# twke18/SPML

Hardware: AMD Instinct MI355X
Metric: images/sec (513x513) + k-means iters/sec (higher is better)
Workload: dtype f32

## Files before the change

### spml_amd/_ffi.py

```python
import ctypes
import os
import threading
from ctypes import c_char_p, c_double, c_float, c_int, c_int64, c_size_t, c_void_p

import torch

_HERE = os.path.dirname(os.path.abspath(__file__))
LIB_PATH = os.environ.get('SPML_HIP_LIB') or os.path.join(_HERE, 'lib', 'libspml_hip.so')

_lib = None
_lock = threading.Lock()

_P = c_void_p
_SIGNATURES = {
    'spml_status_string': (c_char_p, [c_int]),
    'spml_abi_version': (c_int, []),
    'spml_normalize_concat_loc_f32': (c_int, [_P, c_int, c_int, c_int, c_int, _P, _P, _P, _P, _P]),
    'spml_normalize_concat_loc_bwd_f32': (c_int, [_P, c_int, c_int, c_int, c_int, _P, _P, _P, _P, _P, _P]),
    'spml_normalize_concat_local_f32': (c_int, [_P, c_int, c_int, c_int, c_int, _P, c_int, _P, _P, _P, _P]),
    'spml_normalize_concat_local_nhwc_supported': (c_int, [c_int, c_int]),
    'spml_normalize_concat_local_nhwc_f32': (c_int, [_P, c_int, c_int, c_int, c_int, _P, c_int, _P, _P, _P, _P]),
    'spml_normalize_concat_local_nhwc_bwd_f32': (c_int, [_P, c_int, c_int, c_int, c_int, _P, c_int, _P, _P, _P,
                                                         _P, _P]),
    'spml_normalize_concat_local_bwd_f32': (c_int, [_P, c_int, c_int, c_int, c_int, _P, c_int, _P, _P, _P,
                                                    _P, _P]),
    'spml_normalize_rows_f32': (c_int, [_P, c_int64, c_int, _P, _P]),
    'spml_normalize_rows_bwd_f32': (c_int, [_P, _P, c_int64, c_int, _P, _P]),
    'spml_kmeans_init_grid_i64': (c_int, [c_int, c_int, c_int, c_int, _P, _P]),
    'spml_relabel_unique_workspace_bytes': (c_size_t, [c_int64]),
    'spml_relabel_unique_i64': (c_int, [_P, c_int64, _P, _P, c_int64, _P, _P, c_size_t, _P]),
    'spml_kmeans_workspace_bytes': (c_size_t, [c_int64, c_int, c_int, c_int, c_int64]),
    'spml_kmeans_run_f32': (c_int, [_P, c_int64, c_int, _P, c_int, c_int64, c_int, _P, c_int, _P, _P,
                                    c_int, _P, c_size_t, _P]),
    'spml_kmeans_assign_f32': (c_int, [_P, c_int64, c_int, _P, c_int, c_int64, c_int, _P, _P, c_int,
                                       _P, c_size_t, _P]),
    'spml_kmeans_fused_pass_f32': (c_int, [_P, c_int64, c_int, _P, c_int, c_int64, c_int, _P, _P, _P,
                                           c_int, _P, c_size_t, _P]),
    'spml_kmeans_preconvert_f32': (c_int, [_P, c_int64, c_int, _P, c_int, c_int64, c_int, _P, c_size_t,
                                           _P]),
    'spml_kmeans_path_name': (c_char_p, [c_int64, c_int, c_int, c_int, c_int64, c_int, c_int, c_int]),
    'spml_kmeans_profile_layout': (c_int, [c_int64, c_int, c_int, c_int, c_int64, c_int, _P, _P]),
    'spml_kmeans_run_profiled_f32': (c_int, [_P, c_int64, c_int, _P, c_int, c_int64, c_int, _P, c_int,
                                             _P, c_int, _P, c_size_t, _P, c_size_t, _P]),
    'spml_segment_sum_normalize_f32': (c_int, [_P, _P, c_int64, c_int, c_int64, _P, _P, _P]),
    'spml_segment_sum_normalize_bwd_f32': (c_int, [_P, _P, _P, c_int64, c_int, c_int64, _P, _P, c_int, _P]),
    'spml_segment_sum_det_workspace_bytes': (c_size_t, [c_int64, c_int]),
    'spml_segment_sum_normalize_det_f32': (c_int, [_P, _P, c_int64, c_int, c_int64, _P, _P, _P, c_size_t, _P]),
    'spml_set_deterministic': (c_int, [c_int]),
    'spml_get_deterministic': (c_int, []),
    'spml_build_experiment': (c_int, []),
    'spml_segsort_nll_workspace_bytes': (c_size_t, [c_int64, c_int64, c_int]),
    'spml_segsort_nll_fwd_f32': (c_int, [_P, _P, _P, c_int64, _P, _P, c_int64, c_int, c_float, c_int,
                                         _P, _P, _P, c_size_t, _P]),
    'spml_segsort_nll_bwd_f32': (c_int, [_P, _P, _P, c_int64, _P, _P, c_int64, c_int, c_float, c_int,
                                         _P, _P, _P, _P, c_int64, _P, c_size_t, _P]),
    'spml_topk_workspace_bytes': (c_size_t, [c_int64, c_int64, c_int, c_int]),
    'spml_topk_affinity_f32': (c_int, [_P, c_int64, _P, c_int64, c_int, c_int, _P, _P, _P, c_float,
                                       _P, _P, _P, c_size_t, _P]),
    'spml_affinity_workspace_bytes': (c_size_t, [c_int, c_int, c_int64]),
    'spml_affinity_transition_f32': (c_int, [_P, c_int, c_int, c_int64, c_float, c_int, _P, _P, c_size_t,
                                             _P]),
    'spml_bn_workspace_bytes': (c_size_t, [c_int64, c_int]),
    'spml_bn_act_fwd_f32': (c_int, [_P, _P, c_int64, c_int, _P, _P, _P, _P, c_float, c_float, c_int, _P, _P, _P,
                                    _P, c_size_t, _P]),
    'spml_bn_act_bwd_f32': (c_int, [_P, _P, _P, c_int64, c_int, _P, _P, _P, _P, _P, _P, _P, _P, c_size_t, _P]),
    'spml_hl8_from_f32': (c_int, [_P, c_int64, c_int, _P, c_int, _P, _P]),
    'spml_hl8_weight_transposed_f32': (c_int, [_P, c_int, c_int, c_int, _P, _P, _P]),
    'spml_conv_hl8_supported': (c_int, [c_int, c_int, c_int]),
    'spml_conv_hl8_f32': (c_int, [_P, _P, _P, _P, _P, _P, _P, c_int, c_int, c_int, c_int, c_int, c_int, c_int, _P]),
    'spml_conv_hl8_stats_layout': (c_int, [c_int, c_int, c_int, c_int, c_int, c_int, _P, _P]),
    'spml_conv_hl8_stats_f32': (c_int, [_P, _P, _P, _P, _P, _P, _P, c_int, c_int, c_int, c_int, c_int, c_int, c_int, _P]),
    'spml_bn_fwd_hl8_chunks_f32': (c_int, [_P, _P, c_int, c_int, _P, _P, c_int64, c_int, _P, _P, _P, _P, c_float, c_float,
                                           c_int, _P, _P, _P, _P, _P, _P, _P, _P, _P]),
    'spml_conv_wgrad_hl8_supported': (c_int, [c_int, c_int, c_int]),
    'spml_conv_wgrad_workspace_bytes': (c_size_t, [c_int, c_int, c_int, c_int, c_int, c_int]),
    'spml_conv_wgrad_hl8_f32': (c_int, [_P, _P, _P, _P, _P, c_int, c_int, c_int, c_int, c_int, c_int, c_int, _P,
                                        c_size_t, _P]),
    'spml_conv_wgrad_pyramid_hl8_supported': (c_int, [c_int, c_int, c_int]),
    'spml_conv_tap_gather_f32': (c_int, [_P, _P, _P, c_int, c_int, c_int, c_int, c_int, _P, _P]),
    'spml_conv_wgrad_pyramid_workspace_bytes': (c_size_t, [c_int, c_int, c_int, c_int, c_int, c_int]),
    'spml_conv_wgrad_pyramid_hl8_f32': (c_int, [_P, _P, _P, _P, _P, c_int, c_int, c_int, c_int, c_int, c_int, _P, _P,
                                                c_size_t, _P]),
    'spml_bn_stats_ext_f32': (c_int, [_P, c_int64, c_int, _P, _P, _P, _P, _P, c_size_t, _P]),
    'spml_bn_stats_ext_chunks_f32': (c_int, [_P, c_int, c_int, c_int64, c_int, _P, _P, _P, _P, _P]),
    'spml_bn_finalize_f32': (c_int, [_P, _P, c_int, c_double, c_float, c_float, _P, _P, _P, _P]),
    'spml_bn_act_apply_hl8_f32': (c_int, [_P, _P, _P, c_int64, c_int, _P, _P, _P, _P, _P, _P, c_int, _P, _P, _P, _P,
                                          _P]),
    'spml_bn_act_bwd_reduce_ext_f32': (c_int, [_P, _P, _P, _P, c_int64, c_int, _P, _P, _P, _P, _P, _P, c_size_t, _P]),
    'spml_bn_act_bwd_apply_hl8_f32': (c_int, [_P, _P, _P, _P, c_int64, c_int, _P, _P, _P, _P, _P, _P, _P, _P,
                                              c_double, _P, _P, _P, _P, _P, _P]),
    'spml_bn_fwd_hl8_f32': (c_int, [_P, _P, _P, c_int64, c_int, _P, _P, _P, _P, c_float, c_float, c_int, _P, _P, _P, _P,
                                    _P, _P, _P, _P, _P, c_size_t, _P]),
    'spml_bn_bwd_hl8_f32': (c_int, [_P, _P, _P, _P, c_int64, c_int, _P, _P, _P, _P, _P, _P, _P, _P, _P, _P, _P, _P,
                                    c_size_t, _P]),
    'spml_conv_hl8_pyramid_f32': (c_int, [_P, _P, _P, _P, _P, _P, _P, c_int, c_int, c_int, c_int, c_int, c_int, _P,
                                          _P]),
    'spml_hl8_weight_transposed_into_f32': (c_int, [_P, c_int, c_int, c_int, _P, _P, c_int, c_int, _P]),
    'spml_absmax_bound_f32': (c_int, [_P, c_int64, _P, c_int, _P]),
    'spml_hl8_weight_set_f32': (c_int, [_P, _P, _P, _P, c_int, _P, _P, _P, _P]),
    'spml_bn_finalize_ranks_f32': (c_int, [_P, c_int, c_int, c_float, c_float, _P, _P, _P, _P, _P, _P]),
    'spml_conv_hl8_affine_f32': (c_int, [_P, _P, _P, _P, _P, _P, c_int, _P, _P, c_int, c_int, c_int, c_int, c_int,
                                         c_int, c_int, _P]),
    'spml_upsample_ce_supported': (c_int, [c_int]),
    'spml_upsample_ce_workspace_bytes': (c_size_t, [c_int, c_int, c_int]),
    'spml_upsample_ce_fwd_f32': (c_int, [_P, _P, c_int, c_int, c_int, c_int, c_int, c_int, c_int64, _P, _P, _P,
                                         c_size_t, _P]),
    'spml_upsample_ce_bwd_f32': (c_int, [_P, _P, _P, c_int, c_int, c_int, c_int, c_int, c_int, c_int64, _P, _P, _P]),
    'spml_bn_stats_f32': (c_int, [_P, c_int64, c_int, _P, _P, _P, c_size_t, _P]),
    'spml_bn_act_apply_f32': (c_int, [_P, _P, c_int64, c_int, _P, _P, _P, _P, c_int, _P, _P]),
    'spml_bn_act_bwd_reduce_f32': (c_int, [_P, _P, _P, c_int64, c_int, _P, _P, _P, _P, _P, c_size_t, _P]),
    'spml_bn_act_bwd_apply_f32': (c_int, [_P, _P, _P, c_int64, c_int, _P, _P, _P, _P, _P, c_double, _P, _P, _P,
                                          _P]),
    'spml_clock_probe': (c_int, [_P, c_int, _P]),
    'spml_maxpool3x3s2_nhwc_f32': (c_int, [_P, c_int, c_int, c_int, c_int, _P, _P]),
    'spml_window_accumulate_f32': (c_int, [_P, c_int, c_int, c_int, _P, _P, c_int, c_int, c_int, c_int,
                                           _P]),
    'spml_unit_hl8_from_nchw_f32': (c_int, [_P, c_int, c_int, c_int, c_int, _P, _P]),
    'spml_class_head_supported': (c_int, [c_int, c_int]),
    'spml_class_head_accumulate_f32': (c_int, [_P, c_int, c_int, c_int, _P, _P, c_int, _P, c_int, c_int, c_int, c_int,
                                               _P]),
    'spml_argmax_channels_i64': (c_int, [_P, c_int, c_int, c_int, c_int, c_int, _P, _P]),
    'spml_iou_counts_i64': (c_int, [_P, _P, c_int64, c_int, _P, _P]),
    'spml_resample_unit_f32': (c_int, [_P, c_int, c_int, c_int, c_int64, c_int64, c_int64, c_int, c_int, c_int, c_int,
                                       c_int, _P, c_int, c_int, _P]),
    'spml_resample_classes_accumulate_f32': (c_int, [_P, c_int, c_int, c_int, c_int64, c_int64, c_int64, c_int, c_int,
                                                     c_int, c_int, c_int, c_int, _P, _P]),
    'spml_cam_finalize_f32': (c_int, [_P, c_int, c_int64, c_int, c_int, _P, c_int, c_float, _P, _P]),
    'spml_upsample_argmax_i64': (c_int, [_P, c_int, c_int, c_int, c_int, c_int, _P, _P]),
}

EXPORTS = tuple(_SIGNATURES)


class SpmlHipError(RuntimeError):
  pass


ABI_VERSION = 6


def lib():
  global _lib
  if _lib is None:
    with _lock:
      if _lib is None:
        if not os.path.exists(LIB_PATH):
          raise SpmlHipError(
              'libspml_hip.so not found at %s -- build it with `python -m spml_amd._build` '
              '(there is no CPU fallback for the HIP path)' % LIB_PATH)
        handle = ctypes.CDLL(LIB_PATH)
        for name, (res, args) in _SIGNATURES.items():
          try:
            fn = getattr(handle, name)
          except AttributeError:
            raise SpmlHipError('libspml_hip.so does not export %s (stale build? run '
                               '`python -m spml_amd._build --force`)' % name)
          fn.restype = res
          fn.argtypes = args
        got = handle.spml_abi_version()
        if got != ABI_VERSION:
          raise SpmlHipError('libspml_hip.so has ABI version %d, this wrapper was written against %d (stale build? '
                             'run `python -m spml_amd._build --force`)' % (got, ABI_VERSION))
        exp = handle.spml_build_experiment()
        want = (int(os.environ.get('SPML_CONV_EXP') or 0) & 0xffff) | ((int(os.environ.get('SPML_P64_EXP') or 0) & 0xffff) << 16)
        if exp != want:
          raise SpmlHipError('libspml_hip.so is a profiling build (SPML_CONV_EXP=%d, SPML_P64_EXP=%d: kernels that skip work '
                             'and overwrite outputs) but this process asks for (%d, %d) -- rebuild with '
                             '`python -m spml_amd._build`' % (exp & 0xffff, exp >> 16, want & 0xffff, want >> 16))
        if os.environ.get('SPML_DETERMINISTIC', '0') not in ('', '0'):
          handle.spml_set_deterministic(1)
        _lib = handle
  return _lib


def set_deterministic(on):
  return bool(lib().spml_set_deterministic(1 if on else 0))


def deterministic():
  return bool(lib().spml_get_deterministic())


def check(rc, what):
  if rc != 0:
    raise SpmlHipError('%s failed: %s (status %d)' % (
        what, lib().spml_status_string(rc).decode(), rc))


def stream_ptr():
  return c_void_p(torch.cuda.current_stream().cuda_stream)


def ptr(t, dtype=None, allow_none=False):
  if t is None:
    if allow_none:
      return c_void_p(0)
    raise SpmlHipError('missing tensor argument')
  if not t.is_cuda:
    raise SpmlHipError('the HIP path needs GPU tensors (got %s); there is no CPU fallback'
                       % t.device)
  if t.device.index != torch.cuda.current_device():
    raise SpmlHipError('tensor lives on %s but the current device is cuda:%d -- wrap the call in '
                       '`torch.cuda.device(tensor.device)`' % (t.device, torch.cuda.current_device()))
  if not t.is_contiguous():
    raise SpmlHipError('tensor must be contiguous')
  if dtype is not None and t.dtype != dtype:
    raise SpmlHipError('expected dtype %s, got %s' % (dtype, t.dtype))
  return c_void_p(t.data_ptr())


def workspace(nbytes, device):
  n = max(int(nbytes), 16)
  if n > (64 << 20):
    g = min(1 << (n.bit_length() - 4), 256 << 20)
    n = (n + g - 1) // g * g
  return torch.empty((n,), dtype=torch.uint8, device=device)



def k1_channels_last(emb, nl):
  return (emb.dim() == 4 and emb.dtype == torch.float32 and not emb.is_contiguous() and
          emb.is_contiguous(memory_format=torch.channels_last) and
          bool(lib().spml_normalize_concat_local_nhwc_supported(int(emb.shape[1]), int(nl))))


def normalize_concat_loc(emb, loc=None, row_map=None, num_rows=None, want_emb=True,
                         want_loc=True):
  n, c, h, w = emb.shape
  nl = 2 if loc is None else int(loc.shape[-1])
  rows = n * h * w if num_rows is None else int(num_rows)
  out_emb = torch.empty((rows, c), dtype=torch.float32, device=emb.device) if want_emb else None
  out_loc = torch.empty((rows, c + nl), dtype=torch.float32, device=emb.device) if want_loc else None
  if k1_channels_last(emb, nl):
    check(lib().spml_normalize_concat_local_nhwc_f32(
        _ptr_any(emb), n, c, h, w, ptr(loc, torch.float32, True), nl,
        ptr(row_map, torch.int64, True), ptr(out_emb, None, True), ptr(out_loc, None, True),
        stream_ptr()), 'spml_normalize_concat_local_nhwc_f32')
    return out_emb, out_loc
  check(lib().spml_normalize_concat_local_f32(
      ptr(emb, torch.float32), n, c, h, w, ptr(loc, torch.float32, True), nl,
      ptr(row_map, torch.int64, True), ptr(out_emb, None, True), ptr(out_loc, None, True),
      stream_ptr()), 'spml_normalize_concat_local_f32')
  return out_emb, out_loc


def normalize_concat_loc_bwd(emb, loc, row_map, d_out_emb, d_out_loc):
  n, c, h, w = emb.shape
  nl = 2 if loc is None else int(loc.shape[-1])
  d_emb = torch.empty_like(emb)
  if k1_channels_last(emb, nl):
    check(lib().spml_normalize_concat_local_nhwc_bwd_f32(
        _ptr_any(emb), n, c, h, w, ptr(loc, torch.float32, True), nl,
        ptr(row_map, torch.int64, True), ptr(d_out_emb, torch.float32, True),
        ptr(d_out_loc, torch.float32, True), _ptr_any(d_emb), stream_ptr()),
          'spml_normalize_concat_local_nhwc_bwd_f32')
    return d_emb
  check(lib().spml_normalize_concat_local_bwd_f32(
      ptr(emb, torch.float32), n, c, h, w, ptr(loc, torch.float32, True), nl,
      ptr(row_map, torch.int64, True), ptr(d_out_emb, torch.float32, True),
      ptr(d_out_loc, torch.float32, True), ptr(d_emb), stream_ptr()),
        'spml_normalize_concat_local_bwd_f32')
  return d_emb


def normalize_rows(x):
  d = x.shape[-1]
  x2 = x.reshape(-1, d)
  y = torch.empty_like(x2)
  check(lib().spml_normalize_rows_f32(ptr(x2, torch.float32), x2.shape[0], d, ptr(y),
                                      stream_ptr()), 'spml_normalize_rows_f32')
  return y.view(x.shape)


def normalize_rows_bwd(x, dy):
  d = x.shape[-1]
  x2, g2 = x.reshape(-1, d), dy.reshape(-1, d).contiguous()
  dx = torch.empty_like(x2)
  check(lib().spml_normalize_rows_bwd_f32(ptr(x2, torch.float32), ptr(g2, torch.float32),
                                          x2.shape[0], d, ptr(dx), stream_ptr()),
        'spml_normalize_rows_bwd_f32')
  return dx.view(x.shape)


def kmeans_init_grid(h, w, ky, kx, device):
  out = torch.empty((h, w), dtype=torch.int64, device=device)
  check(lib().spml_kmeans_init_grid_i64(h, w, ky, kx, ptr(out), stream_ptr()),
        'spml_kmeans_init_grid_i64')
  return out


_last_kmeans = None


def relabel_unique(keys, with_uniq=True, padded=False):
  keys = keys.reshape(-1)
  if keys.dtype != torch.int64 or not keys.is_contiguous():
    keys = keys.long().contiguous()
  p = keys.shape[0]
  inv = torch.empty((p,), dtype=torch.int64, device=keys.device)
  count = torch.empty((1,), dtype=torch.int64, device=keys.device)
  if padded:
    uniq = torch.full((p,), torch.iinfo(torch.int64).max, dtype=torch.int64, device=keys.device)
  else:
    uniq = torch.empty((p if with_uniq else 0,), dtype=torch.int64, device=keys.device)
  ws = workspace(lib().spml_relabel_unique_workspace_bytes(p), keys.device)
  check(lib().spml_relabel_unique_i64(ptr(keys, torch.int64, p == 0), p, ptr(inv, allow_none=p == 0),
                                      ptr(uniq, allow_none=uniq.numel() == 0), uniq.numel(), ptr(count), ptr(ws),
                                      ws.numel(), stream_ptr()), 'spml_relabel_unique_i64')
  if padded:
    return uniq, inv, count
  if not with_uniq:
    return None, inv, count
  return uniq[:int(count.item())], inv, count


def _note_kmeans(p, d, k, n_img, max_seg_len, iterations, given, flags):
  global _last_kmeans
  _last_kmeans = (int(p), int(d), int(k), int(n_img), int(max_seg_len), int(iterations), int(given),
                  int(flags))


def kmeans_path_name(p, d, k, n_img, max_seg_len, iterations, given_centroids=False, flags=0):
  return lib().spml_kmeans_path_name(int(p), int(d), int(k), int(n_img), int(max_seg_len),
                                     int(iterations), int(bool(given_centroids)), int(flags)).decode()


def kmeans_last_path():
  return 'none' if _last_kmeans is None else lib().spml_kmeans_path_name(*_last_kmeans).decode()


def kmeans_run(x, seg_offsets, max_seg_len, k, labels_init, iterations, want_centroids=False,
               flags=0):
  p, d = x.shape
  n_img = seg_offsets.shape[0] - 1
  labels = torch.empty((p,), dtype=torch.int64, device=x.device)
  cent = (torch.zeros((n_img, k, d), dtype=torch.float32, device=x.device)
          if want_centroids else None)
  nbytes = lib().spml_kmeans_workspace_bytes(p, d, k, n_img, max_seg_len)
  ws = workspace(nbytes, x.device)
  check(lib().spml_kmeans_run_f32(
      ptr(x, torch.float32), p, d, ptr(seg_offsets, torch.int64), n_img, int(max_seg_len), k,
      ptr(labels_init, torch.int64), int(iterations), ptr(labels), ptr(cent, None, True),
      int(flags), ptr(ws), ws.numel(), stream_ptr()), 'spml_kmeans_run_f32')
  _note_kmeans(p, d, k, n_img, max_seg_len, iterations, 0, flags)
  return (labels, cent) if want_centroids else labels


def kmeans_run_profiled(x, seg_offsets, max_seg_len, k, labels_init, iterations, flags=0):
  import ctypes
  p, d = x.shape
  n_img = seg_offsets.shape[0] - 1
  n_pass, wgs = ctypes.c_int(0), ctypes.c_int(0)
  check(lib().spml_kmeans_profile_layout(p, d, k, n_img, int(max_seg_len), int(iterations),
                                         ctypes.byref(n_pass), ctypes.byref(wgs)),
        'spml_kmeans_profile_layout')
  clocks = torch.zeros((n_pass.value, wgs.value, 2), dtype=torch.int64, device=x.device)
  labels = torch.empty((p,), dtype=torch.int64, device=x.device)
  ws = workspace(lib().spml_kmeans_workspace_bytes(p, d, k, n_img, max_seg_len), x.device)
  check(lib().spml_kmeans_run_profiled_f32(
      ptr(x, torch.float32), p, d, ptr(seg_offsets, torch.int64), n_img, int(max_seg_len), k,
      ptr(labels_init, torch.int64), int(iterations), ptr(labels), int(flags), ptr(ws), ws.numel(),
      ptr(clocks), clocks.numel(), stream_ptr()), 'spml_kmeans_run_profiled_f32')
  _note_kmeans(p, d, k, n_img, max_seg_len, iterations, 0, flags)
  c = clocks.cpu()
  start = torch.where(c[:, :, 0] == 0, torch.full_like(c[:, :, 0], torch.iinfo(torch.int64).max), c[:, :, 0])
  dur = (c[:, :, 1].max(dim=1).values - start.min(dim=1).values).double() * 0.01
  return labels, dur


def kmeans_assign(x, seg_offsets, max_seg_len, centroids, flags=0):
  p, d = x.shape
  n_img = seg_offsets.shape[0] - 1
  k = centroids.shape[-2]
  labels = torch.empty((p,), dtype=torch.int64, device=x.device)
  nbytes = lib().spml_kmeans_workspace_bytes(p, d, k, n_img, max_seg_len)
  ws = workspace(nbytes, x.device)
  check(lib().spml_kmeans_assign_f32(
      ptr(x, torch.float32), p, d, ptr(seg_offsets, torch.int64), n_img, int(max_seg_len), k,
      ptr(centroids, torch.float32), ptr(labels), int(flags), ptr(ws), ws.numel(),
      stream_ptr()), 'spml_kmeans_assign_f32')
  _note_kmeans(p, d, k, n_img, max_seg_len, 1, 1, flags)
  return labels


def kmeans_workspace(x, seg_offsets, max_seg_len, k):
  p, d = x.shape
  return workspace(lib().spml_kmeans_workspace_bytes(p, d, k, seg_offsets.shape[0] - 1, max_seg_len),
                   x.device)


def kmeans_preconvert(x, seg_offsets, max_seg_len, k, ws):
  p, d = x.shape
  check(lib().spml_kmeans_preconvert_f32(
      ptr(x, torch.float32), p, d, ptr(seg_offsets, torch.int64), seg_offsets.shape[0] - 1,
      int(max_seg_len), int(k), ptr(ws), ws.numel(), stream_ptr()), 'spml_kmeans_preconvert_f32')


def kmeans_fused_pass(x, seg_offsets, max_seg_len, centroids, ws=None, preconverted=False, flags=0,
                      out=None):
  p, d = x.shape
  n_img = seg_offsets.shape[0] - 1
  k = centroids.shape[-2]
  if ws is None:
    ws = kmeans_workspace(x, seg_offsets, max_seg_len, k)
  if out is None:
    out = (torch.empty((p,), dtype=torch.int64, device=x.device),
           torch.empty((n_img, k, d), dtype=torch.float32, device=x.device))
  labels, sums = out
  flags = int(flags) | (32 if preconverted else 0)
  check(lib().spml_kmeans_fused_pass_f32(
      ptr(x, torch.float32), p, d, ptr(seg_offsets, torch.int64), n_img, int(max_seg_len), k,
      ptr(centroids, torch.float32), ptr(labels, torch.int64), ptr(sums, torch.float32), flags,
      ptr(ws), ws.numel(), stream_ptr()), 'spml_kmeans_fused_pass_f32')
  _note_kmeans(p, d, k, n_img, max_seg_len, 1, 1, flags)
  return labels, sums


def clock_probe(device, spin_us, stream):
  out = torch.zeros((2,), dtype=torch.int64, device=device)
  stream.wait_stream(torch.cuda.current_stream(device))
  check(lib().spml_clock_probe(ptr(out), int(spin_us), c_void_p(stream.cuda_stream)), 'spml_clock_probe')
  return out


def maxpool3x3s2_nhwc(x):
  n, c, h, w = x.shape
  oh, ow = (h - 1) // 2 + 1, (w - 1) // 2 + 1
  y = torch.empty((n, c, oh, ow), dtype=torch.float32, device=x.device, memory_format=torch.channels_last)
  check(lib().spml_maxpool3x3s2_nhwc_f32(_ptr_any(x), n, h, w, c, _ptr_any(y), stream_ptr()), 'spml_maxpool3x3s2_nhwc_f32')
  return y


def segment_sum_normalize(x, ids, m):
  p, d = x.shape
  sums = torch.empty((m, d), dtype=torch.float32, device=x.device)
  protos = torch.empty((m, d), dtype=torch.float32, device=x.device)
  if deterministic():
    nbytes = lib().spml_segment_sum_det_workspace_bytes(int(m), d)
    ws = workspace(nbytes, x.device)
    check(lib().spml_segment_sum_normalize_det_f32(ptr(x, torch.float32), ptr(ids, torch.int64), p, d, int(m),
                                                   ptr(sums), ptr(protos), ptr(ws), ws.numel(), stream_ptr()),
          'spml_segment_sum_normalize_det_f32')
    return protos, sums
  check(lib().spml_segment_sum_normalize_f32(ptr(x, torch.float32), ptr(ids, torch.int64), p, d,
                                             int(m), ptr(sums), ptr(protos), stream_ptr()),
        'spml_segment_sum_normalize_f32')
  return protos, sums


def segment_sum_normalize_bwd(d_protos, sums, ids, p):
  m, d = sums.shape
  scratch = torch.empty_like(sums)
  dx = torch.empty((p, d), dtype=torch.float32, device=sums.device)
  check(lib().spml_segment_sum_normalize_bwd_f32(
      ptr(d_protos, torch.float32), ptr(sums, torch.float32), ptr(ids, torch.int64), p, d, m,
      ptr(scratch), ptr(dx), 0, stream_ptr()), 'spml_segment_sum_normalize_bwd_f32')
  return dx


def segsort_nll_fwd(emb, own, px_code, protos, pr_code, kappa, mode):
  p, d = emb.shape
  m = protos.shape[0]
  nll = torch.empty((p,), dtype=torch.float32, device=emb.device)
  stats = torch.empty((p, 4), dtype=torch.float32, device=emb.device)
  ws = workspace(lib().spml_segsort_nll_workspace_bytes(p, m, d), emb.device)
  check(lib().spml_segsort_nll_fwd_f32(
      ptr(emb, torch.float32), ptr(own, torch.int64), ptr(px_code, torch.int64), p,
      ptr(protos, torch.float32), ptr(pr_code, torch.int64), m, d, float(kappa), int(mode),
      ptr(nll), ptr(stats), ptr(ws), ws.numel(), stream_ptr()), 'spml_segsort_nll_fwd_f32')
  return nll, stats


def segsort_nll_bwd(emb, own, px_code, protos, pr_code, kappa, mode, stats, d_nll, m_grad=-1):
  p, d = emb.shape
  m = protos.shape[0]
  d_emb = torch.empty_like(emb)
  d_protos = torch.zeros_like(protos)
  ws = workspace(lib().spml_segsort_nll_workspace_bytes(p, m, d), emb.device)
  check(lib().spml_segsort_nll_bwd_f32(
      ptr(emb, torch.float32), ptr(own, torch.int64), ptr(px_code, torch.int64), p,
      ptr(protos, torch.float32), ptr(pr_code, torch.int64), m, d, float(kappa), int(mode),
      ptr(stats, torch.float32), ptr(d_nll, torch.float32), ptr(d_emb), ptr(d_protos),
      int(m_grad), ptr(ws), ws.numel(), stream_ptr()), 'spml_segsort_nll_bwd_f32')
  return d_emb, d_protos


def topk_affinity(q, protos, k, q_group=None, pr_group=None, pr_valid=None, masked_value=-2.0):
  nq, d = q.shape
  m = protos.shape[0]
  idx = torch.empty((nq, k), dtype=torch.int64, device=q.device)
  val = torch.empty((nq, k), dtype=torch.float32, device=q.device)
  ws = workspace(lib().spml_topk_workspace_bytes(nq, m, d, k), q.device)
  check(lib().spml_topk_affinity_f32(
      ptr(q, torch.float32), nq, ptr(protos, torch.float32), m, d, int(k),
      ptr(q_group, torch.int64, True), ptr(pr_group, torch.int64, True),
      ptr(pr_valid, torch.uint8, True), float(masked_value), ptr(idx), ptr(val), ptr(ws),
      ws.numel(), stream_ptr()), 'spml_topk_affinity_f32')
  return idx, val


def window_accumulate(patch, acc, counts, sh, sw):
  c, h, w = patch.shape
  big_c, big_h, big_w = acc.shape
  if big_c != c or tuple(counts.shape) != (big_h, big_w):
    raise SpmlHipError('window_accumulate: shape mismatch')
  check(lib().spml_window_accumulate_f32(
      ptr(patch, torch.float32), c, h, w, ptr(acc, torch.float32), ptr(counts, torch.float32),
      big_h, big_w, int(sh), int(sw), stream_ptr()), 'spml_window_accumulate_f32')


def unit_hl8_from_nchw(x):
  n, c, h, w = x.shape
  out = torch.empty((n * h * w * c * 4,), dtype=torch.uint8, device=x.device)
  check(lib().spml_unit_hl8_from_nchw_f32(ptr(x, torch.float32), n, c, h, w, ptr(out), stream_ptr()),
        'spml_unit_hl8_from_nchw_f32')
  return Hl8(out, torch.ones((1,), dtype=torch.float32, device=x.device), n * h * w, c)


def class_head_supported(ch, ncls):
  return bool(lib().spml_class_head_supported(int(ch), int(ncls)))


def class_head_accumulate(hidden, weight, bias, canvas, sh, sw, h, w):
  ncls, ch = weight.shape
  if hidden.numel() != h * w * ch or canvas.dim() != 3 or canvas.shape[0] != ncls or bias.numel() != ncls:
    raise SpmlHipError('class_head_accumulate: shape mismatch')
  check(lib().spml_class_head_accumulate_f32(
      _ptr_any(hidden), ch, int(h), int(w), ptr(weight, torch.float32), ptr(bias, torch.float32), ncls,
      ptr(canvas, torch.float32), canvas.shape[1], canvas.shape[2], int(sh), int(sw), stream_ptr()),
        'spml_class_head_accumulate_f32')


def argmax_channels(canvas, h, w):
  ncls, hp, wp = canvas.shape
  out = torch.empty((h, w), dtype=torch.int64, device=canvas.device)
  check(lib().spml_argmax_channels_i64(ptr(canvas, torch.float32), ncls, hp, wp, int(h), int(w), ptr(out),
                                       stream_ptr()), 'spml_argmax_channels_i64')
  return out


def iou_counts(pred, target, ncls, counts=None):
  if pred.numel() != target.numel():
    raise SpmlHipError('iou_counts: pred and target differ in size')
  if counts is None:
    counts = torch.zeros((3, ncls), dtype=torch.int64, device=pred.device)
  elif tuple(counts.shape) != (3, ncls):
    raise SpmlHipError('iou_counts: counts must be [3, num_classes]')
  check(lib().spml_iou_counts_i64(ptr(pred, torch.int64), ptr(target, torch.int64), pred.numel(), int(ncls),
                                  ptr(counts, torch.int64), stream_ptr()), 'spml_iou_counts_i64')
  return counts


COMBINE_MODES = {'prob_mean': 0, 'logit_mean': 1}


def _combine(combine):
  if combine not in COMBINE_MODES:
    raise SpmlHipError("combine must be 'prob_mean' or 'logit_mean' (got %r)" % (combine,))
  return COMBINE_MODES[combine]


def _view_args(x, crop_hw, out_hw, what):
  if x.dim() != 3:
    raise SpmlHipError('%s: expected a [C, Hp, Wp] tensor' % what)
  c, hp, wp = x.shape
  (rh, rw), (oh, ow) = crop_hw, out_hw
  if not (0 < rh <= hp and 0 < rw <= wp and oh > 0 and ow > 0):
    raise SpmlHipError('%s: crop %r / output %r do not fit a %d x %d plane' % (what, crop_hw, out_hw, hp, wp))
  sc, sy, sx = x.stride()
  return c, hp, wp, sc, sy, sx, int(rh), int(rw), int(oh), int(ow)


def resample_unit(emb, crop_hw, flip, out_hw, out, b):
  c, hp, wp, sc, sy, sx, rh, rw, oh, ow = _view_args(emb, crop_hw, out_hw, 'resample_unit')
  if out.dim() != 3 or out.shape[1] != c or out.shape[2] != oh * ow or not 0 <= b < out.shape[0]:
    raise SpmlHipError('resample_unit: out must be [B, %d, %d] with b < B' % (c, oh * ow))
  check(lib().spml_resample_unit_f32(_ptr_any(emb), c, hp, wp, sc, sy, sx, rh, rw, int(bool(flip)), oh, ow,
                                     ptr(out, torch.float32), out.shape[0], int(b), stream_ptr()),
        'spml_resample_unit_f32')
  return out


def resample_classes_accumulate(logit, crop_hw, flip, out_hw, acc, combine='prob_mean'):
  ncls, hp, wp, sc, sy, sx, rh, rw, oh, ow = _view_args(logit, crop_hw, out_hw, 'resample_classes_accumulate')
  if acc.shape[0] != ncls or acc.numel() != ncls * oh * ow:
    raise SpmlHipError('resample_classes_accumulate: acc must hold [%d, %d] values' % (ncls, oh * ow))
  check(lib().spml_resample_classes_accumulate_f32(_ptr_any(logit), ncls, hp, wp, sc, sy, sx, rh, rw, int(bool(flip)),
                                                   oh, ow, _combine(combine), ptr(acc, torch.float32), stream_ptr()),
        'spml_resample_classes_accumulate_f32')
  return acc


def cam_finalize(acc, num_views, label_tags, combine='prob_mean', background_threshold=None):
  ncls = acc.shape[0]
  if label_tags.numel() != ncls or label_tags.dtype not in (torch.bool, torch.uint8):
    raise SpmlHipError('cam_finalize: label_tags must be a bool [%d] tensor' % ncls)
  if int(num_views) < 1:
    raise SpmlHipError('cam_finalize: no views')
  cam = torch.empty_like(acc)
  tags = label_tags.view(torch.uint8) if label_tags.dtype == torch.bool else label_tags
  check(lib().spml_cam_finalize_f32(ptr(acc, torch.float32), ncls, acc.numel() // ncls, int(num_views),
                                    _combine(combine), ptr(tags, torch.uint8), int(background_threshold is not None),
                                    float(background_threshold or 0.0), ptr(cam), stream_ptr()),
        'spml_cam_finalize_f32')
  return cam


def upsample_argmax(cam, h, w):
  if cam.dim() != 3:
    raise SpmlHipError('upsample_argmax: expected [ncls, oh, ow]')
  ncls, oh, ow = cam.shape
  out = torch.empty((int(h), int(w)), dtype=torch.int64, device=cam.device)
  check(lib().spml_upsample_argmax_i64(ptr(cam, torch.float32), ncls, oh, ow, int(h), int(w), ptr(out), stream_ptr()),
        'spml_upsample_argmax_i64')
  return out


def affinity_transition(emb, scale=5.0, power=20):
  b, c, n = emb.shape
  trans = torch.empty((n, n), dtype=torch.float32, device=emb.device)
  ws = workspace(lib().spml_affinity_workspace_bytes(b, c, n), emb.device)
  check(lib().spml_affinity_transition_f32(
      ptr(emb, torch.float32), b, c, n, float(scale), int(power), ptr(trans), ptr(ws), ws.numel(),
      stream_ptr()), 'spml_affinity_transition_f32')
  return trans


def _nhwc_rows(t):
  if t.dim() == 2:
    return t.shape[0], t.shape[1]
  n, c, h, w = t.shape
  if not t.is_contiguous(memory_format=torch.channels_last):
    raise SpmlHipError('fused batch norm needs channels-last (NHWC) tensors')
  return n * h * w, c


def _ptr_any(t, allow_none=False):
  if t is None:
    if allow_none:
      return c_void_p(0)
    raise SpmlHipError('missing tensor argument')
  if not t.is_cuda or t.dtype != torch.float32:
    raise SpmlHipError('expected a float32 GPU tensor (got %s on %s)' % (t.dtype, t.device))
  if t.device.index != torch.cuda.current_device():
    raise SpmlHipError('tensor lives on %s but the current device is cuda:%d' % (t.device, torch.cuda.current_device()))
  return c_void_p(t.data_ptr())


_bn_ws = {}


def _bn_workspace(r, c, device):
  need = lib().spml_bn_workspace_bytes(r, c)
  key = (device.index, torch.cuda.current_stream().cuda_stream)
  ws = _bn_ws.get(key)
  if ws is None or ws.numel() < need:
    ws = workspace(need, device)
    _bn_ws[key] = ws
  return ws


def bn_act_fwd(x, residual, gamma, beta, running_mean, running_var, momentum, eps, relu):
  r, c = _nhwc_rows(x)
  y = torch.empty_like(x)
  stats = torch.empty((2, c), dtype=torch.float32, device=x.device)
  ws = _bn_workspace(r, c, x.device)
  check(lib().spml_bn_act_fwd_f32(
      _ptr_any(x), _ptr_any(residual, True), r, c, ptr(gamma, torch.float32), ptr(beta, torch.float32),
      ptr(running_mean, None, True), ptr(running_var, None, True), float(momentum), float(eps),
      int(bool(relu)), _ptr_any(y), c_void_p(stats[0].data_ptr()), c_void_p(stats[1].data_ptr()), ptr(ws),
      ws.numel(), stream_ptr()), 'spml_bn_act_fwd_f32')
  return y, stats[0], stats[1]


def bn_act_bwd(dy, y, x, mean, invstd, gamma, want_dx=True, want_dres=False):
  r, c = _nhwc_rows(dy)
  dx = torch.empty_like(dy) if want_dx else None
  dres = torch.empty_like(dy) if want_dres else None
  dgb = torch.empty((2, c), dtype=torch.float32, device=dy.device)
  ws = _bn_workspace(r, c, dy.device)
  check(lib().spml_bn_act_bwd_f32(
      _ptr_any(dy), _ptr_any(y, True), _ptr_any(x), r, c, c_void_p(mean.data_ptr()), c_void_p(invstd.data_ptr()),
      ptr(gamma, torch.float32), c_void_p(dgb[0].data_ptr()), c_void_p(dgb[1].data_ptr()), _ptr_any(dx, True),
      _ptr_any(dres, True), ptr(ws), ws.numel(), stream_ptr()), 'spml_bn_act_bwd_f32')
  return dx, dres, dgb[0], dgb[1]


def bn_stats(x):
  r, c = _nhwc_rows(x)
  mean = torch.empty((c,), dtype=torch.float32, device=x.device)
  m2 = torch.empty((c,), dtype=torch.float32, device=x.device)
  ws = workspace(lib().spml_bn_workspace_bytes(r, c), x.device)
  check(lib().spml_bn_stats_f32(_ptr_any(x), r, c, ptr(mean), ptr(m2), ptr(ws), ws.numel(), stream_ptr()),
        'spml_bn_stats_f32')
  return mean, m2


def bn_act_apply(x, residual, mean, invstd, gamma, beta, relu):
  r, c = _nhwc_rows(x)
  y = torch.empty_like(x)
  check(lib().spml_bn_act_apply_f32(_ptr_any(x), _ptr_any(residual, True), r, c, ptr(mean), ptr(invstd),
                                    ptr(gamma, torch.float32), ptr(beta, torch.float32), int(bool(relu)),
                                    _ptr_any(y), stream_ptr()), 'spml_bn_act_apply_f32')
  return y


def bn_act_bwd_reduce(dy, y, x, mean, invstd):
  r, c = _nhwc_rows(x)
  s0 = torch.empty((c,), dtype=torch.float32, device=x.device)
  s1 = torch.empty((c,), dtype=torch.float32, device=x.device)
  ws = workspace(lib().spml_bn_workspace_bytes(r, c), x.device)
  check(lib().spml_bn_act_bwd_reduce_f32(_ptr_any(dy), _ptr_any(y, True), _ptr_any(x), r, c, ptr(mean),
                                         ptr(invstd), ptr(s0), ptr(s1), ptr(ws), ws.numel(), stream_ptr()),
        'spml_bn_act_bwd_reduce_f32')
  return s0, s1


def bn_act_bwd_apply(dy, y, x, mean, invstd, gamma, sum_dz, sum_dz_xhat, count, want_dx=True,
                     want_dres=False):
  r, c = _nhwc_rows(dy)
  count, count_dev = _count_args(count)
  dx = torch.empty_like(dy) if want_dx else None
  dres = torch.empty_like(dy) if want_dres else None
  check(lib().spml_bn_act_bwd_apply_f32(
      _ptr_any(dy), _ptr_any(y, True), _ptr_any(x, True), r, c, ptr(mean, None, True), ptr(invstd, None, True),
      ptr(gamma, None, True), ptr(sum_dz, None, True), ptr(sum_dz_xhat, None, True), count, count_dev,
      _ptr_any(dx, True), _ptr_any(dres, True), stream_ptr()), 'spml_bn_act_bwd_apply_f32')
  return dx, dres



class Hl8(object):
  __slots__ = ('data', 'bound', 'rows', 'channels')

  def __init__(self, data, bound, rows, channels):
    self.data, self.bound, self.rows, self.channels = data, bound, rows, channels


def hl8_from_f32(x, rows=None, channels=None, bound=None):
  if rows is None:
    rows, channels = _nhwc_rows(x)
  compute = bound is None
  if compute:
    bound = torch.empty((1,), dtype=torch.float32, device=x.device)
  out = torch.empty((rows * channels * 4,), dtype=torch.uint8, device=x.device)
  check(lib().spml_hl8_from_f32(_ptr_any(x), rows, channels, c_void_p(bound.data_ptr()), int(compute),
                                ptr(out), stream_ptr()), 'spml_hl8_from_f32')
  return Hl8(out, bound, rows, channels)


def hl8_weight(w):
  cout, cin, kh, kw = w.shape
  taps = kh * kw
  wl = w.detach().contiguous(memory_format=torch.channels_last)
  fwd = hl8_from_f32(wl, cout, taps * cin)
  tr = torch.empty((cout * taps * cin * 4,), dtype=torch.uint8, device=w.device)
  check(lib().spml_hl8_weight_transposed_f32(_ptr_any(wl), cout, taps, cin, c_void_p(fwd.bound.data_ptr()),
                                             ptr(tr), stream_ptr()), 'spml_hl8_weight_transposed_f32')
  return fwd, Hl8(tr, fwd.bound, cin, taps * cout)


def conv_hl8_supported(k, n, taps):
  return bool(lib().spml_conv_hl8_supported(int(k), int(n), int(taps)))


def conv_hl8(a, b, n_img, h, w, taps, dilation=1, addend=None, addend_mask=None):
  k, n = a.channels, b.rows
  if a.rows != n_img * h * w or b.channels != taps * k:
    raise SpmlHipError('conv_hl8: operand shapes do not match')
  out = torch.empty((n_img, n, h, w), dtype=torch.float32, device=a.data.device,
                    memory_format=torch.channels_last)
  check(lib().spml_conv_hl8_f32(ptr(a.data), c_void_p(a.bound.data_ptr()), ptr(b.data),
                                c_void_p(b.bound.data_ptr()), _ptr_any(addend, True), _dp(addend_mask), _ptr_any(out),
                                n_img, h, w,
                                k, n, taps, dilation, stream_ptr()), 'spml_conv_hl8_f32')
  return out


class ChunkStats(object):

  def __init__(self, data, chunks, chunk_rows, bound):
    self.data, self.chunks, self.chunk_rows, self.bound = data, chunks, chunk_rows, bound


def conv_hl8_stats(a, b, n_img, h, w, taps, dilation=1):
  import ctypes
  k, n = a.channels, b.rows
  chunks, rows = ctypes.c_int(0), ctypes.c_int(0)
  if os.environ.get('SPML_CONV_BN_STATS') == '0' or lib().spml_conv_hl8_stats_layout(
      n_img, h, w, k, n, taps, ctypes.byref(chunks), ctypes.byref(rows)) != 0:
    return conv_hl8(a, b, n_img, h, w, taps, dilation), None
  if a.rows != n_img * h * w or b.channels != taps * k:
    raise SpmlHipError('conv_hl8_stats: operand shapes do not match')
  dev = a.data.device
  out = torch.empty((n_img, n, h, w), dtype=torch.float32, device=dev, memory_format=torch.channels_last)
  st = torch.empty((4, chunks.value, n), dtype=torch.float32, device=dev)
  bound = _f32(1, dev)
  check(lib().spml_conv_hl8_stats_f32(ptr(a.data), c_void_p(a.bound.data_ptr()), ptr(b.data),
                                      c_void_p(b.bound.data_ptr()), _ptr_any(out), _dp(st), _dp(bound), n_img, h, w,
                                      k, n, taps, dilation, stream_ptr()), 'spml_conv_hl8_stats_f32')
  return out, ChunkStats(st, chunks.value, rows.value, bound)


def conv_wgrad_hl8_supported(k, n, taps):
  return bool(lib().spml_conv_wgrad_hl8_supported(int(k), int(n), int(taps)))


_wgrad_ws = {}


def conv_wgrad_hl8(dy, x, n_img, h, w, taps, dilation=1):
  n, k = dy.channels, x.channels
  if dy.rows != n_img * h * w or x.rows != dy.rows:
    raise SpmlHipError('conv_wgrad_hl8: operand shapes do not match')
  need = lib().spml_conv_wgrad_workspace_bytes(n_img, h, w, k, n, taps)
  key = (dy.data.device.index, torch.cuda.current_stream().cuda_stream)
  ws = _wgrad_ws.get(key)
  if ws is None or ws.numel() < need:
    ws = workspace(need, dy.data.device)
    _wgrad_ws[key] = ws
  side = 3 if taps == 9 else 1
  dw = torch.empty((n, k, side, side), dtype=torch.float32, device=dy.data.device,
                   memory_format=torch.channels_last)
  check(lib().spml_conv_wgrad_hl8_f32(ptr(dy.data), c_void_p(dy.bound.data_ptr()), ptr(x.data),
                                      c_void_p(x.bound.data_ptr()), _ptr_any(dw), n_img, h, w, k, n, taps,
                                      dilation, ptr(ws), ws.numel(), stream_ptr()), 'spml_conv_wgrad_hl8_f32')
  return dw


def conv_wgrad_pyramid_hl8_supported(k, n, branches):
  return bool(lib().spml_conv_wgrad_pyramid_hl8_supported(int(k), int(n), int(branches)))


def conv_wgrad_pyramid_hl8(dy, x, n_img, h, w, dilations):
  n, k, nb = dy.channels, x.channels, len(dilations)
  if dy.rows != n_img * h * w or x.rows != dy.rows:
    raise SpmlHipError('conv_wgrad_pyramid_hl8: operand shapes do not match')
  need = lib().spml_conv_wgrad_pyramid_workspace_bytes(n_img, h, w, k, n, nb)
  if need == 0:
    raise SpmlHipError('conv_wgrad_pyramid_hl8: unsupported shape (K %d, N %d, %d branches)' % (k, n, nb))
  key = (dy.data.device.index, torch.cuda.current_stream().cuda_stream)
  ws = _wgrad_ws.get(key)
  if ws is None or ws.numel() < need:
    ws = workspace(need, dy.data.device)
    _wgrad_ws[key] = ws
  dw = torch.empty((nb, n, 3, 3, k), dtype=torch.float32, device=dy.data.device)
  dil = (ctypes.c_int * nb)(*[int(d) for d in dilations])
  check(lib().spml_conv_wgrad_pyramid_hl8_f32(ptr(dy.data), c_void_p(dy.bound.data_ptr()), ptr(x.data),
                                              c_void_p(x.bound.data_ptr()), _ptr_any(dw), n_img, h, w, k, n, nb,
                                              ctypes.cast(dil, c_void_p), ptr(ws), ws.numel(), stream_ptr()),
        'spml_conv_wgrad_pyramid_hl8_f32')
  return [dw[b].permute(0, 3, 1, 2) for b in range(nb)]


def _f32(n, device):
  return torch.empty((n,), dtype=torch.float32, device=device)


def _dp(t):
  return c_void_p(0) if t is None else c_void_p(t.data_ptr())


def bn_stats_ext(x, rows, channels, chunk_stats=None):
  st = torch.empty((5, channels), dtype=torch.float32, device=x.device)
  st[0].fill_(float(rows))
  if chunk_stats is not None:
    check(lib().spml_bn_stats_ext_chunks_f32(_dp(chunk_stats.data), chunk_stats.chunks, chunk_stats.chunk_rows, rows,
                                             channels, _dp(st[1]), _dp(st[2]), _dp(st[3]), _dp(st[4]), stream_ptr()),
          'spml_bn_stats_ext_chunks_f32')
    return st
  ws = _bn_workspace(rows, channels, x.device)
  check(lib().spml_bn_stats_ext_f32(_ptr_any(x), rows, channels, _dp(st[1]), _dp(st[2]), _dp(st[3]), _dp(st[4]),
                                    ptr(ws), ws.numel(), stream_ptr()), 'spml_bn_stats_ext_f32')
  return st


def _count_args(count):
  if torch.is_tensor(count):
    return 0.0, ptr(count, torch.float32)
  return float(count), None


def bn_finalize_ranks(gathered, eps, momentum, running_mean, running_var):
  world, _, c = gathered.shape
  out = torch.empty((2 * c + 4,), dtype=torch.float32, device=gathered.device)
  mean, invstd, total = out[:c], out[c:2 * c], out[2 * c:2 * c + 1]
  check(lib().spml_bn_finalize_ranks_f32(ptr(gathered, torch.float32), world, c, float(eps), float(momentum),
                                         _dp(running_mean), _dp(running_var), _dp(mean), _dp(invstd), _dp(total),
                                         stream_ptr()),
        'spml_bn_finalize_ranks_f32')
  return mean, invstd, total


def bn_finalize(mean, m2, count, eps, momentum, running_mean, running_var):
  invstd = torch.empty_like(mean)
  check(lib().spml_bn_finalize_f32(_dp(mean), _dp(m2), mean.numel(), float(count), float(eps), float(momentum),
                                   _dp(running_mean), _dp(running_var), _dp(invstd), stream_ptr()),
        'spml_bn_finalize_f32')
  return invstd


def bn_act_apply_hl8(x, rows, channels, residual, residual_bound, mean, invstd, gamma, beta, cmax, cmin, relu,
                     want_f32, want_hl8, like=None, want_mask=False):
  y = torch.empty_like(x if like is None else like) if want_f32 else None
  yh = torch.empty((rows * channels * 4,), dtype=torch.uint8, device=x.device) if want_hl8 else None
  bound = _f32(1, x.device)
  mask = torch.empty((rows * (channels // 4),), dtype=torch.uint8, device=x.device) if want_mask else None
  check(lib().spml_bn_act_apply_hl8_f32(
      _ptr_any(x), _ptr_any(residual, True), _dp(residual_bound), rows, channels, _dp(mean), _dp(invstd),
      ptr(gamma, torch.float32), ptr(beta, torch.float32), _dp(cmax), _dp(cmin), int(bool(relu)), _ptr_any(y, True),
      _dp(yh), _dp(bound), _dp(mask), stream_ptr()), 'spml_bn_act_apply_hl8_f32')
  return y, (Hl8(yh, bound, rows, channels) if want_hl8 else None), bound, mask


def bn_act_bwd_reduce_ext(dy, y, relu_mask, x, rows, channels, mean, invstd):
  st = torch.empty((3, channels), dtype=torch.float32, device=dy.device)
  ws = _bn_workspace(rows, channels, dy.device)
  check(lib().spml_bn_act_bwd_reduce_ext_f32(
      _ptr_any(dy), _ptr_any(y, True), _dp(relu_mask), _ptr_any(x), rows, channels,
      _dp(mean), _dp(invstd), _dp(st[0]), _dp(st[1]), _dp(st[2]), ptr(ws), ws.numel(), stream_ptr()),
        'spml_bn_act_bwd_reduce_ext_f32')
  return st


def bn_act_bwd_apply_hl8(dy, y, relu_mask, x, rows, channels, mean, invstd, gamma, s0, s1, max_dz, cmax, cmin, count,
                         want_dx_f32=False, want_dx_hl8=True, want_dres=False):
  dx = torch.empty_like(dy) if want_dx_f32 else None
  dxh = torch.empty((rows * channels * 4,), dtype=torch.uint8, device=dy.device) if want_dx_hl8 else None
  bound = _f32(1, dy.device) if want_dx_hl8 else None
  dres = torch.empty_like(dy) if want_dres else None
  count, count_dev = _count_args(count)
  check(lib().spml_bn_act_bwd_apply_hl8_f32(
      _ptr_any(dy), _ptr_any(y, True), _dp(relu_mask), _ptr_any(x), rows, channels,
      _dp(mean), _dp(invstd), ptr(gamma, torch.float32), _dp(s0), _dp(s1), _dp(max_dz), _dp(cmax), _dp(cmin),
      count, count_dev, _ptr_any(dx, True), _dp(dxh), _dp(bound), _ptr_any(dres, True), stream_ptr()),
        'spml_bn_act_bwd_apply_hl8_f32')
  return dx, (Hl8(dxh, bound, rows, channels) if want_dx_hl8 else None), dres


def bn_fwd_hl8(x, rows, channels, residual, residual_bound, gamma, beta, running_mean, running_var, momentum, eps,
               relu, want_f32, want_hl8, want_mask, chunk_stats=None):
  y = torch.empty_like(x) if want_f32 else None
  yh = torch.empty((rows * channels * 4,), dtype=torch.uint8, device=x.device) if want_hl8 else None
  bound = _f32(1, x.device) if chunk_stats is None else chunk_stats.bound
  mask = torch.empty((rows * (channels // 4),), dtype=torch.uint8, device=x.device) if want_mask else None
  st = torch.empty((4, channels), dtype=torch.float32, device=x.device)
  if chunk_stats is not None:
    check(lib().spml_bn_fwd_hl8_chunks_f32(
        _ptr_any(x), _dp(chunk_stats.data), chunk_stats.chunks, chunk_stats.chunk_rows, _ptr_any(residual, True),
        _dp(residual_bound), rows, channels, ptr(gamma, torch.float32), ptr(beta, torch.float32), _dp(running_mean),
        _dp(running_var), float(momentum), float(eps), int(bool(relu)), _ptr_any(y, True), _dp(yh), _dp(bound),
        _dp(mask), _dp(st[0]), _dp(st[1]), _dp(st[2]), _dp(st[3]), stream_ptr()), 'spml_bn_fwd_hl8_chunks_f32')
    return y, (Hl8(yh, bound, rows, channels) if want_hl8 else None), bound, mask, (st[0], st[1], st[2], st[3])
  ws = _bn_workspace(rows, channels, x.device)
  check(lib().spml_bn_fwd_hl8_f32(
      _ptr_any(x), _ptr_any(residual, True), _dp(residual_bound), rows, channels, ptr(gamma, torch.float32),
      ptr(beta, torch.float32), _dp(running_mean), _dp(running_var), float(momentum), float(eps), int(bool(relu)),
      _ptr_any(y, True), _dp(yh), _dp(bound), _dp(mask), _dp(st[0]), _dp(st[1]), _dp(st[2]), _dp(st[3]), ptr(ws),
      ws.numel(), stream_ptr()), 'spml_bn_fwd_hl8_f32')
  return y, (Hl8(yh, bound, rows, channels) if want_hl8 else None), bound, mask, (st[0], st[1], st[2], st[3])


def bn_bwd_hl8(dy, relu_mask, x, rows, channels, saved, gamma, want_dres=False):
  mean, invstd, cmax, cmin = saved
  dxh = torch.empty((rows * channels * 4,), dtype=torch.uint8, device=dy.device)
  bound = _f32(1, dy.device)
  dres = torch.empty_like(dy) if want_dres else None
  dgb = torch.empty((2, channels), dtype=torch.float32, device=dy.device)
  ws = _bn_workspace(rows, channels, dy.device)
  check(lib().spml_bn_bwd_hl8_f32(
      _ptr_any(dy), c_void_p(0), _dp(relu_mask), _ptr_any(x), rows, channels, _dp(mean), _dp(invstd),
      ptr(gamma, torch.float32), _dp(cmax), _dp(cmin), _dp(dgb[0]), _dp(dgb[1]), c_void_p(0), _dp(dxh), _dp(bound),
      _ptr_any(dres, True), ptr(ws), ws.numel(), stream_ptr()), 'spml_bn_bwd_hl8_f32')
  return Hl8(dxh, bound, rows, channels), dres, dgb[0], dgb[1]


def conv_hl8_pyramid_dgrad(dy, weights, dilations, n_img, h, w):
  groups = len(weights)
  cout, cin = weights[0].shape[0], weights[0].shape[1]
  dev = dy.data.device
  bound = torch.empty((1,), dtype=torch.float32, device=dev)
  wl = [wt.detach().contiguous(memory_format=torch.channels_last) for wt in weights]
  for g, wt in enumerate(wl):
    check(lib().spml_absmax_bound_f32(_ptr_any(wt), wt.numel(), _dp(bound), int(g == 0), stream_ptr()),
          'spml_absmax_bound_f32')
  b = torch.empty((cin * 9 * groups * cout * 4,), dtype=torch.uint8, device=dev)
  for g, wt in enumerate(wl):
    check(lib().spml_hl8_weight_transposed_into_f32(_ptr_any(wt), cout, 9, cin, _dp(bound), ptr(b), 9 * groups, 9 * g,
                                                    stream_ptr()), 'spml_hl8_weight_transposed_into_f32')
  out = torch.empty((n_img, cin, h, w), dtype=torch.float32, device=dev, memory_format=torch.channels_last)
  import ctypes
  dil = (ctypes.c_int * 4)(*([int(d) for d in dilations] + [1] * (4 - groups)))
  check(lib().spml_conv_hl8_pyramid_f32(ptr(dy.data), _dp(dy.bound), ptr(b), _dp(bound), c_void_p(0), c_void_p(0),
                                        _ptr_any(out), n_img, h, w, cout, cin, groups, dil, stream_ptr()),
        'spml_conv_hl8_pyramid_f32')
  return out


def conv_hl8_pyramid_forward(x, weights, biases, dilations, n_img, h, w):
  import ctypes
  groups = len(weights)
  cout, cin = weights[0].shape[0], weights[0].shape[1]
  dev = x.data.device
  cat = torch.cat([wt.detach().permute(0, 2, 3, 1).reshape(cout, 9 * cin) for wt in weights], dim=1).contiguous()
  b = hl8_from_f32(cat, cout, 9 * groups * cin)
  bias = None
  if any(bb is not None for bb in biases):
    bias = sum(bb.detach() for bb in biases if bb is not None).contiguous()
  out = torch.empty((n_img, cout, h, w), dtype=torch.float32, device=dev, memory_format=torch.channels_last)
  dil = (ctypes.c_int * 4)(*([int(d) for d in dilations] + [1] * (4 - groups)))
  check(lib().spml_conv_hl8_pyramid_f32(ptr(x.data), _dp(x.bound), ptr(b.data), _dp(b.bound), _dp(bias), c_void_p(0),
                                        _ptr_any(out), n_img, h, w, cin, cout, groups, dil, stream_ptr()),
        'spml_conv_hl8_pyramid_f32')
  return out


_pyramid_operand_cache = {}


def conv_hl8_pyramid_forward_gemm_supported(cin, cout, groups):
  return (16 <= cout <= 1024 and cout & (cout - 1) == 0 and 1 <= groups <= 4 and
          conv_hl8_supported(cin, 9 * groups * cout, 1))


def conv_hl8_pyramid_forward_gemm(x, weights, biases, dilations, n_img, h, w):
  import ctypes
  groups = len(weights)
  cout, cin = weights[0].shape[0], weights[0].shape[1]
  dev = x.data.device
  import weakref
  refs, vers = _pyramid_operand_cache.get('refs', ()), _pyramid_operand_cache.get('versions', ())
  if (len(refs) == groups and all(r() is wt for r, wt in zip(refs, weights)) and
      vers == tuple(wt._version for wt in weights)):
    operand = _pyramid_operand_cache['operand']
  else:
    cat = torch.stack([wt.detach().permute(2, 3, 0, 1).reshape(9 * cout, cin) for wt in weights]).reshape(
        9 * groups * cout, cin).contiguous()
    operand = hl8_from_f32(cat, 9 * groups * cout, cin)
    _pyramid_operand_cache.update(refs=tuple(weakref.ref(wt) for wt in weights),
                                  versions=tuple(wt._version for wt in weights), operand=operand)
  z = conv_hl8(x, operand, n_img, h, w, 1)
  bias = None
  if any(bb is not None for bb in biases):
    bias = sum(bb.detach() for bb in biases if bb is not None).contiguous()
  out = torch.empty((n_img, cout, h, w), dtype=torch.float32, device=dev, memory_format=torch.channels_last)
  dil = (ctypes.c_int * groups)(*[int(d) for d in dilations])
  check(lib().spml_conv_tap_gather_f32(_ptr_any(z), _dp(bias), _ptr_any(out), n_img, h, w, cout, groups,
                                       ctypes.cast(dil, c_void_p), stream_ptr()), 'spml_conv_tap_gather_f32')
  return out


def hl8_weight_set(weights):
  import ctypes
  n = len(weights)
  dev = weights[0].device
  wl = [wt.detach().contiguous(memory_format=torch.channels_last) for wt in weights]
  bounds = torch.empty((4,), dtype=torch.float32, device=dev)
  shapes = [(wt.shape[0], wt.shape[1], wt.shape[2] * wt.shape[3]) for wt in wl]
  fwd = [torch.empty((co * ci * t * 4,), dtype=torch.uint8, device=dev) for co, ci, t in shapes]
  tr = [torch.empty((co * ci * t * 4,), dtype=torch.uint8, device=dev) for co, ci, t in shapes]
  pv, iv = ctypes.c_void_p * n, ctypes.c_int * n
  check(lib().spml_hl8_weight_set_f32(
      pv(*[wt.data_ptr() for wt in wl]), iv(*[sh[0] for sh in shapes]), iv(*[sh[1] for sh in shapes]),
      iv(*[sh[2] for sh in shapes]), n, _dp(bounds), pv(*[t.data_ptr() for t in fwd]),
      pv(*[t.data_ptr() for t in tr]), stream_ptr()), 'spml_hl8_weight_set_f32')
  out = []
  for i, (co, ci, t) in enumerate(shapes):
    b = bounds[i:i + 1]
    out.append((Hl8(fwd[i], b, co, t * ci), Hl8(tr[i], b, ci, t * co)))
  return out


def conv_hl8_affine(a, b, bias, n_img, h, w, taps, dilation=1, addend=None, relu=True, want_hl8=True):
  k, n = a.channels, b.rows
  if a.rows != n_img * h * w or b.channels != taps * k:
    raise SpmlHipError('conv_hl8_affine: operand shapes do not match')
  dev = a.data.device
  out = torch.empty((n_img, n, h, w), dtype=torch.float32, device=dev, memory_format=torch.channels_last)
  bound = _f32(1, dev) if want_hl8 else None
  check(lib().spml_conv_hl8_affine_f32(ptr(a.data), _dp(a.bound), ptr(b.data), _dp(b.bound), ptr(bias, torch.float32),
                                       _ptr_any(addend, True), int(bool(relu)), _ptr_any(out), _dp(bound), n_img, h, w,
                                       k, n, taps, dilation, stream_ptr()), 'spml_conv_hl8_affine_f32')
  return out, (hl8_from_f32(out, bound=bound) if want_hl8 else None)


def upsample_ce_supported(c):
  return bool(lib().spml_upsample_ce_supported(int(c)))


def upsample_ce_fwd(logits_nhwc, labels, ignore_index):
  n, h, w, c = logits_nhwc.shape
  hh, ww = labels.shape[-2:]
  lse = torch.empty((n, hh, ww), dtype=torch.float32, device=logits_nhwc.device)
  result = torch.empty((3,), dtype=torch.float32, device=logits_nhwc.device)
  ws = workspace(lib().spml_upsample_ce_workspace_bytes(n, hh, ww), logits_nhwc.device)
  check(lib().spml_upsample_ce_fwd_f32(ptr(logits_nhwc, torch.float32), ptr(labels, torch.int64), n, c, h, w, hh, ww,
                                       int(ignore_index), ptr(lse), ptr(result), ptr(ws), ws.numel(), stream_ptr()),
        'spml_upsample_ce_fwd_f32')
  return result, lse


def upsample_ce_bwd(logits_nhwc, labels, lse, ignore_index, scale):
  n, h, w, c = logits_nhwc.shape
  hh, ww = labels.shape[-2:]
  d = torch.empty_like(logits_nhwc)
  check(lib().spml_upsample_ce_bwd_f32(ptr(logits_nhwc, torch.float32), ptr(labels, torch.int64),
                                       ptr(lse, torch.float32), n, c, h, w, hh, ww, int(ignore_index),
                                       ptr(scale, torch.float32), ptr(d), stream_ptr()), 'spml_upsample_ce_bwd_f32')
  return d
```

### spml_amd/csrc/bn_act.hip

```cpp
#include "common.hpp"

namespace spml {
namespace {


__device__ __forceinline__ float4v relu_mask_bits(float4v dz, const unsigned char* __restrict__ mask, size_t row,
                                                  int C, int q) {
  const unsigned m = mask[row * (size_t)(C >> 2) + q];
#pragma unroll
  for (int e = 0; e < 4; ++e) dz[e] = (m >> e) & 1u ? dz[e] : 0.f;
  return dz;
}

__device__ __forceinline__ float bn_pow2_scale(float bound) {
  if (!(bound > 0.f) || bound > 1e38f) return 1.f;
  int e;
  (void)frexpf(bound, &e);
  e = 14 - e;
  e = e < -100 ? -100 : (e > 100 ? 100 : e);
  return ldexpf(1.f, e);
}

__device__ __forceinline__ void store_hl8_quad(uint2* __restrict__ out, size_t row, int C, int q, float4v v,
                                               float s) {
  union { uint2 u; _Float16 h[4]; } hh, ll;
#pragma unroll
  for (int e = 0; e < 4; ++e) {
    const float x = v[e] * s;
    const _Float16 h = (_Float16)x;
    hh.h[e] = h;
    ll.h[e] = (_Float16)(x - (float)h);
  }
  const bool odd = (q & 1) != 0;
  const uint2 send = odd ? hh.u : ll.u;
  uint2 recv;
  recv.x = (unsigned)__shfl_xor((int)send.x, 1, kWave);
  recv.y = (unsigned)__shfl_xor((int)send.y, 1, kWave);
  uint4 unit;
  if (odd) { unit.x = recv.x; unit.y = recv.y; unit.z = ll.u.x; unit.w = ll.u.y; }
  else { unit.x = hh.u.x; unit.y = hh.u.y; unit.z = recv.x; unit.w = recv.y; }
  reinterpret_cast<uint4*>(out)[(row * (size_t)(C >> 3) + (q >> 1)) * 2 + (odd ? 1 : 0)] = unit;
}

template <int MODE, int MASK>
__global__ __launch_bounds__(256) void bn_partial(const float* __restrict__ x, const float* __restrict__ dy,
                                                  const float* __restrict__ y, const float* __restrict__ mean,
                                                  int64_t R, int C, int cq, int chunk_rows,
                                                  float* __restrict__ pa, float* __restrict__ pb,
                                                  const unsigned char* __restrict__ yh, float* __restrict__ pc,
                                                  float* __restrict__ pd, float* __restrict__ zero_me) {
  if (zero_me && blockIdx.x == 0 && blockIdx.y == 0 && threadIdx.x == 0) *zero_me = 0.f;
  __shared__ float4v sa[256], sb[256];
  const int tx = threadIdx.x % cq, ty = threadIdx.x / cq, nty = 256 / cq;
  const int q = blockIdx.x * cq + tx;
  const int64_t r0 = (int64_t)blockIdx.y * chunk_rows;
  const int nrows = (int)min((int64_t)chunk_rows, R - r0);
  const int cquads = C >> 2;
  float4v a = {0.f, 0.f, 0.f, 0.f}, b = {0.f, 0.f, 0.f, 0.f};
  float4v mu = {0.f, 0.f, 0.f, 0.f};
  float4v hi = {-3.4e38f, -3.4e38f, -3.4e38f, -3.4e38f}, lo = {3.4e38f, 3.4e38f, 3.4e38f, 3.4e38f};
  if (MODE == 1) hi = a;
  if (q < cquads) {
    mu = MODE == 1 ? *reinterpret_cast<const float4v*>(mean + 4 * q)
                   : *reinterpret_cast<const float4v*>(x + (size_t)r0 * C + 4 * q);
#pragma unroll 4
    for (int r = ty; r < nrows; r += nty) {
      const size_t o = (size_t)(r0 + r) * C + 4 * q;
      const float4v xv = *reinterpret_cast<const float4v*>(x + o);
      if (MODE == 0) {
        const float4v d = xv - mu;
        a += d;
        b += d * d;
#pragma unroll
        for (int e = 0; e < 4; ++e) { hi[e] = fmaxf(hi[e], xv[e]); lo[e] = fminf(lo[e], xv[e]); }
      } else {
        float4v dz = *reinterpret_cast<const float4v*>(dy + o);
        if (MASK == 1) {
          const float4v yv = *reinterpret_cast<const float4v*>(y + o);
#pragma unroll
          for (int e = 0; e < 4; ++e) dz[e] = yv[e] > 0.f ? dz[e] : 0.f;
        } else if (MASK == 2) {
          dz = relu_mask_bits(dz, yh, (size_t)(r0 + r), C, q);
        }
        a += dz;
        b += dz * (xv - mu);
#pragma unroll
        for (int e = 0; e < 4; ++e) hi[e] = fmaxf(hi[e], fabsf(dz[e]));
      }
    }
  }
  sa[threadIdx.x] = a;
  sb[threadIdx.x] = b;
  __syncthreads();
  if (ty == 0 && q < cquads) {
    for (int i = 1; i < nty; ++i) { a += sa[i * cq + tx]; b += sb[i * cq + tx]; }
    if (MODE == 0) {
      const float inv = 1.0f / (float)nrows;
      const float4v m = a * inv;
      b = b - m * m * (float)nrows;
#pragma unroll
      for (int e = 0; e < 4; ++e) b[e] = fmaxf(b[e], 0.f);
      a = m + mu;
    }
    *reinterpret_cast<float4v*>(pa + (size_t)blockIdx.y * C + 4 * q) = a;
    *reinterpret_cast<float4v*>(pb + (size_t)blockIdx.y * C + 4 * q) = b;
  }
  if (pc) {
    __syncthreads();
    sa[threadIdx.x] = hi;
    sb[threadIdx.x] = lo;
    __syncthreads();
    if (ty == 0 && q < cquads) {
      for (int i = 1; i < nty; ++i) {
#pragma unroll
        for (int e = 0; e < 4; ++e) {
          hi[e] = fmaxf(hi[e], sa[i * cq + tx][e]);
          lo[e] = fminf(lo[e], sb[i * cq + tx][e]);
        }
      }
      *reinterpret_cast<float4v*>(pc + (size_t)blockIdx.y * C + 4 * q) = hi;
      if (MODE == 0) *reinterpret_cast<float4v*>(pd + (size_t)blockIdx.y * C + 4 * q) = lo;
    }
  }
}

struct BnFinal { int fin; float eps, momentum; float* running_mean; float* running_var; };
struct BnBound {
  float* bound;
  const float* res_bound;
  const float* gamma;
  const float* beta;
  const float* mean;
  const float* cmax;
  const float* cmin;
  float inv_count;
};
constexpr int kMergeLanes = 64, kMergeCh = 4;

__device__ inline float merge_lanes(float v, float* sh, int tx, int ty) {
  __syncthreads();
  sh[ty * kMergeCh + tx] = v;
  __syncthreads();
  float t = 0.f;
#pragma unroll 16
  for (int i = 0; i < kMergeLanes; ++i) t += sh[i * kMergeCh + tx];
  return t;
}

template <int MODE>
__global__ __launch_bounds__(kMergeCh * kMergeLanes) void bn_merge(
    const float* __restrict__ pa, const float* __restrict__ pb, int64_t R, int C, int chunks, int chunk_rows,
    const float* __restrict__ invstd, float* __restrict__ out_a, float* __restrict__ out_b, BnFinal f,
    const float* __restrict__ pc, const float* __restrict__ pd, float* __restrict__ out_c,
    float* __restrict__ out_d, BnBound bb) {
  __shared__ float sh[kMergeCh * kMergeLanes];
  __shared__ float sh_bound[kMergeCh];
  const int tx = threadIdx.x % kMergeCh, ty = threadIdx.x / kMergeCh;
  const int n_live = min(kMergeCh, C - (int)blockIdx.x * kMergeCh);
  auto publish_bound = [&](float v) {
    sh_bound[tx] = v;
    __builtin_amdgcn_wave_barrier();
    if (tx == 0) {
      unsigned m = __float_as_uint(v);
      for (int i = 1; i < n_live; ++i) m = max(m, __float_as_uint(sh_bound[i]));
      atomicMax(reinterpret_cast<unsigned*>(bb.bound), m);
    }
  };
  const int c = min(blockIdx.x * kMergeCh + tx, C - 1);
  const bool live = blockIdx.x * kMergeCh + tx < C && ty == 0;
  float hi = -3.4e38f, lo = 3.4e38f;
  constexpr int kMergeRegs = 16;
  const bool in_regs = chunks <= kMergeRegs * kMergeLanes;
  const bool ext = pc && out_c;
  float ra[kMergeRegs], rb[kMergeRegs], rc[kMergeRegs], rd[kMergeRegs];
  if (in_regs) {
#pragma unroll
    for (int j = 0; j < kMergeRegs; ++j) {
      const int i = ty + j * kMergeLanes;
      const bool ok = i < chunks;
      const size_t o = (size_t)(ok ? i : 0) * C + c;
      ra[j] = ok ? pa[o] : 0.f;
      rb[j] = ok ? pb[o] : 0.f;
      rc[j] = (ok && ext) ? pc[o] : -3.4e38f;
      rd[j] = (ok && ext && MODE == 0) ? pd[o] : 3.4e38f;
    }
  }
  float p_gamma = 0.f, p_beta = 0.f, p_res = 0.f, p_rm = 0.f, p_rv = 0.f, p_is = 0.f, p_mu = 0.f, p_cmax = 0.f, p_cmin = 0.f;
  if (live) {
    if (MODE == 0) {
      if (f.fin && bb.bound) { p_gamma = bb.gamma[c]; p_beta = bb.beta[c]; p_res = bb.res_bound ? *bb.res_bound : 0.f; }
      if (f.fin && f.running_mean) { p_rm = f.running_mean[c]; p_rv = f.running_var[c]; }
    } else {
      p_is = invstd[c];
      if (bb.bound) { p_mu = bb.mean[c]; p_cmax = bb.cmax[c]; p_cmin = bb.cmin[c]; p_gamma = bb.gamma[c]; }
    }
  }
  if (ext) {
    if (in_regs) {
#pragma unroll
      for (int j = 0; j < kMergeRegs; ++j) {
        hi = fmaxf(hi, rc[j]);
        if (MODE == 0) lo = fminf(lo, rd[j]);
      }
    } else {
#pragma unroll 4
      for (int i = ty; i < chunks; i += kMergeLanes) {
        hi = fmaxf(hi, pc[(size_t)i * C + c]);
        if (MODE == 0) lo = fminf(lo, pd[(size_t)i * C + c]);
      }
    }
    __syncthreads();
    sh[ty * kMergeCh + tx] = hi;
    __syncthreads();
    for (int i = 0; i < kMergeLanes; ++i) hi = fmaxf(hi, sh[i * kMergeCh + tx]);
    if (MODE == 0) {
      __syncthreads();
      sh[ty * kMergeCh + tx] = lo;
      __syncthreads();
      for (int i = 0; i < kMergeLanes; ++i) lo = fminf(lo, sh[i * kMergeCh + tx]);
    }
    if (live) {
      out_c[c] = hi;
      if (MODE == 0) out_d[c] = lo;
    }
  }
  if (MODE == 0) {
    float sm = 0.f;
    if (in_regs) {
#pragma unroll
      for (int j = 0; j < kMergeRegs; ++j) {
        const int i = ty + j * kMergeLanes;
        if (i < chunks) {
          const float nb = (float)min((int64_t)chunk_rows, R - (int64_t)i * chunk_rows);
          sm += ra[j] * nb;
        }
      }
    } else {
#pragma unroll 4
      for (int i = ty; i < chunks; i += kMergeLanes) {
        const float nb = (float)min((int64_t)chunk_rows, R - (int64_t)i * chunk_rows);
        sm += pa[(size_t)i * C + c] * nb;
      }
    }
    const float m = merge_lanes(sm, sh, tx, ty) / (float)R;
    float m2 = 0.f;
    if (in_regs) {
#pragma unroll
      for (int j = 0; j < kMergeRegs; ++j) {
        const int i = ty + j * kMergeLanes;
        if (i < chunks) {
          const float nb = (float)min((int64_t)chunk_rows, R - (int64_t)i * chunk_rows);
          const float d = ra[j] - m;
          m2 += rb[j] + d * d * nb;
        }
      }
    } else {
#pragma unroll 4
      for (int i = ty; i < chunks; i += kMergeLanes) {
        const float nb = (float)min((int64_t)chunk_rows, R - (int64_t)i * chunk_rows);
        const float d = pa[(size_t)i * C + c] - m;
        m2 += pb[(size_t)i * C + c] + d * d * nb;
      }
    }
    m2 = merge_lanes(m2, sh, tx, ty);
    if (!live) return;
    out_a[c] = m;
    if (f.fin) {
      const float is = 1.0f / sqrtf(m2 / (float)R + f.eps);
      out_b[c] = is;
      if (bb.bound) {
        const float sc = p_gamma * is, b = p_beta;
        const float v = fmaxf(fabsf((hi - m) * sc + b), fabsf((lo - m) * sc + b)) * 1.0001f + p_res;
        publish_bound(v);
      }
      if (f.running_mean) {
        f.running_mean[c] = (1.f - f.momentum) * p_rm + f.momentum * m;
        f.running_var[c] = (1.f - f.momentum) * p_rv +
                           f.momentum * (m2 / (float)(R > 1 ? R - 1 : 1));
      }
    } else {
      out_b[c] = m2;
    }
  } else {
    float s0 = 0.f, s1 = 0.f;
    if (in_regs) {
#pragma unroll
      for (int j = 0; j < kMergeRegs; ++j)
        if (ty + j * kMergeLanes < chunks) { s0 += ra[j]; s1 += rb[j]; }
    } else {
      for (int i = ty; i < chunks; i += kMergeLanes) { s0 += pa[(size_t)i * C + c]; s1 += pb[(size_t)i * C + c]; }
    }
    s0 = merge_lanes(s0, sh, tx, ty);
    s1 = merge_lanes(s1, sh, tx, ty);
    if (!live) return;
    out_a[c] = s0;
    out_b[c] = s1 * p_is;
    if (bb.bound) {
      const float is = p_is, mu = p_mu;
      const float xh = fmaxf(fabsf(p_cmax - mu), fabsf(p_cmin - mu)) * is;
      const float v = fabsf(p_gamma * is) *
                      (hi + fabsf(s0) * bb.inv_count + xh * fabsf(s1 * is) * bb.inv_count) * 1.0001f;
      publish_bound(v);
    }
  }
}


template <bool HAS_RES>
__global__ __launch_bounds__(256) void bn_apply(const float* __restrict__ x, const float* __restrict__ res,
                                                int64_t R, int C, int cq, int apply_rows,
                                                const float* __restrict__ mean,
                                                const float* __restrict__ invstd,
                                                const float* __restrict__ gamma,
                                                const float* __restrict__ beta, int relu,
                                                float* __restrict__ y, uint2* __restrict__ yh,
                                                const float* __restrict__ ybound,
                                                unsigned char* __restrict__ mask) {
  const int tx = threadIdx.x % cq, ty = threadIdx.x / cq, nty = 256 / cq;
  const int q = blockIdx.x * cq + tx;
  if (q >= (C >> 2)) return;
  const float ys = yh ? bn_pow2_scale(*ybound) : 1.f;
  const float4v mu = *reinterpret_cast<const float4v*>(mean + 4 * q);
  const float4v sc = *reinterpret_cast<const float4v*>(invstd + 4 * q) *
                     *reinterpret_cast<const float4v*>(gamma + 4 * q);
  const float4v sh = *reinterpret_cast<const float4v*>(beta + 4 * q);
  const int64_t r0 = (int64_t)blockIdx.y * apply_rows;
  const int64_t r1 = min(R, r0 + apply_rows);
#pragma unroll 4
  for (int64_t r = r0 + ty; r < r1; r += nty) {
    const size_t o = (size_t)r * C + 4 * q;
    float4v v = (*reinterpret_cast<const float4v*>(x + o) - mu) * sc + sh;
    if (HAS_RES) v += *reinterpret_cast<const float4v*>(res + o);
    if (relu) {
#pragma unroll
      for (int e = 0; e < 4; ++e) v[e] = fmaxf(v[e], 0.f);
    }
    if (y) *reinterpret_cast<float4v*>(y + o) = v;
    if (yh) store_hl8_quad(yh, (size_t)r, C, q, v, ys);
    if (mask)
      mask[(size_t)r * (C >> 2) + q] = (unsigned char)((v[0] > 0.f) | ((v[1] > 0.f) << 1) | ((v[2] > 0.f) << 2) |
                                                       ((v[3] > 0.f) << 3));
  }
}

template <int MASK>
__global__ __launch_bounds__(256) void bn_bwd_apply(const float* __restrict__ dy, const float* __restrict__ y,
                                                    const float* __restrict__ x, int64_t R, int C, int cq,
                                                    int apply_rows, const float* __restrict__ mean,
                                                    const float* __restrict__ invstd,
                                                    const float* __restrict__ gamma,
                                                    const float* __restrict__ sum_dz,
                                                    const float* __restrict__ sum_dz_xhat, float inv_count,
                                                    const float* __restrict__ count_dev,
                                                    float* __restrict__ dx, float* __restrict__ dres,
                                                    const unsigned char* __restrict__ yh, uint2* __restrict__ dxh,
                                                    const float* __restrict__ dxbound) {
  const int tx = threadIdx.x % cq, ty = threadIdx.x / cq, nty = 256 / cq;
  const int q = blockIdx.x * cq + tx;
  if (q >= (C >> 2)) return;
  if (count_dev) inv_count = 1.f / count_dev[0];
  const float ds = dxh ? bn_pow2_scale(*dxbound) : 1.f;
  float4v mu = {0.f, 0.f, 0.f, 0.f}, is = mu, gi = mu, c0 = mu, c1 = mu;
  if (dx || dxh) {
    mu = *reinterpret_cast<const float4v*>(mean + 4 * q);
    is = *reinterpret_cast<const float4v*>(invstd + 4 * q);
    gi = *reinterpret_cast<const float4v*>(gamma + 4 * q) * is;
    c0 = *reinterpret_cast<const float4v*>(sum_dz + 4 * q) * inv_count;
    c1 = *reinterpret_cast<const float4v*>(sum_dz_xhat + 4 * q) * inv_count;
  }
  const int64_t r0 = (int64_t)blockIdx.y * apply_rows;
  const int64_t r1 = min(R, r0 + apply_rows);
#pragma unroll 4
  for (int64_t r = r0 + ty; r < r1; r += nty) {
    const size_t o = (size_t)r * C + 4 * q;
    float4v dz = *reinterpret_cast<const float4v*>(dy + o);
    if (MASK == 1) {
      const float4v yv = *reinterpret_cast<const float4v*>(y + o);
#pragma unroll
      for (int e = 0; e < 4; ++e) dz[e] = yv[e] > 0.f ? dz[e] : 0.f;
    } else if (MASK == 2) {
      dz = relu_mask_bits(dz, yh, (size_t)r, C, q);
    }
    if (dres) *reinterpret_cast<float4v*>(dres + o) = dz;
    if (dx || dxh) {
      const float4v xh = (*reinterpret_cast<const float4v*>(x + o) - mu) * is;
      const float4v g = gi * (dz - c0 - xh * c1);
      if (dx) *reinterpret_cast<float4v*>(dx + o) = g;
      if (dxh) store_hl8_quad(dxh, (size_t)r, C, q, g, ds);
    }
  }
}

__device__ __forceinline__ float block_max_256(float v, float* sh) {
#pragma unroll
  for (int o = 32; o > 0; o >>= 1) v = fmaxf(v, __shfl_xor(v, o, kWave));
  if ((threadIdx.x & 63) == 0) sh[threadIdx.x >> 6] = v;
  __syncthreads();
  return fmaxf(fmaxf(sh[0], sh[1]), fmaxf(sh[2], sh[3]));
}

__global__ __launch_bounds__(256) void bn_bound_fwd(int C, const float* __restrict__ cmax,
                                                    const float* __restrict__ cmin,
                                                    const float* __restrict__ mean,
                                                    const float* __restrict__ invstd,
                                                    const float* __restrict__ gamma,
                                                    const float* __restrict__ beta,
                                                    const float* __restrict__ res_bound, float* __restrict__ out) {
  __shared__ float sh[4];
  float m = 0.f;
  for (int c = threadIdx.x; c < C; c += 256) {
    const float sc = gamma[c] * invstd[c];
    m = fmaxf(m, fmaxf(fabsf((cmax[c] - mean[c]) * sc + beta[c]), fabsf((cmin[c] - mean[c]) * sc + beta[c])));
  }
  m = block_max_256(m, sh);
  if (threadIdx.x == 0) out[0] = m * 1.0001f + (res_bound ? res_bound[0] : 0.f);
}

__global__ __launch_bounds__(256) void bn_bound_bwd(int C, const float* __restrict__ max_dz,
                                                    const float* __restrict__ cmax,
                                                    const float* __restrict__ cmin,
                                                    const float* __restrict__ mean,
                                                    const float* __restrict__ invstd,
                                                    const float* __restrict__ gamma,
                                                    const float* __restrict__ sum_dz,
                                                    const float* __restrict__ sum_dz_xhat, float inv_count,
                                                    const float* __restrict__ count_dev,
                                                    float* __restrict__ out) {
  __shared__ float sh[4];
  float m = 0.f;
  if (count_dev) inv_count = 1.f / count_dev[0];
  for (int c = threadIdx.x; c < C; c += 256) {
    const float xh = fmaxf(fabsf(cmax[c] - mean[c]), fabsf(cmin[c] - mean[c])) * invstd[c];
    m = fmaxf(m, fabsf(gamma[c] * invstd[c]) *
                     (max_dz[c] + fabsf(sum_dz[c]) * inv_count + xh * fabsf(sum_dz_xhat[c]) * inv_count));
  }
  m = block_max_256(m, sh);
  if (threadIdx.x == 0) out[0] = m * 1.0001f;
}

__global__ __launch_bounds__(256) void bn_finalize(int C, const float* __restrict__ mean,
                                                   const float* __restrict__ m2, float count, float eps,
                                                   float momentum, float* __restrict__ running_mean,
                                                   float* __restrict__ running_var, float* __restrict__ invstd) {
  const int c = blockIdx.x * 256 + threadIdx.x;
  if (c >= C) return;
  invstd[c] = 1.0f / sqrtf(m2[c] / count + eps);
  if (running_mean) {
    running_mean[c] = (1.f - momentum) * running_mean[c] + momentum * mean[c];
    running_var[c] = (1.f - momentum) * running_var[c] + momentum * (m2[c] / (count > 1.f ? count - 1.f : 1.f));
  }
}

__global__ __launch_bounds__(256) void bn_finalize_ranks(int C, int world, const float* __restrict__ stats,
                                                         float eps, float momentum,
                                                         float* __restrict__ running_mean,
                                                         float* __restrict__ running_var,
                                                         float* __restrict__ mean_out,
                                                         float* __restrict__ invstd,
                                                         float* __restrict__ total_out) {
  const int c = blockIdx.x * 256 + threadIdx.x;
  if (c >= C) return;
  float total = 0.f, sm = 0.f;
  for (int r = 0; r < world; ++r) {
    const float n = stats[((size_t)r * 3 + 0) * C + c];
    total += n;
    sm += n * stats[((size_t)r * 3 + 1) * C + c];
  }
  const float m = sm / total;
  float m2 = 0.f;
  for (int r = 0; r < world; ++r) {
    const float n = stats[((size_t)r * 3 + 0) * C + c];
    const float d = stats[((size_t)r * 3 + 1) * C + c] - m;
    m2 += stats[((size_t)r * 3 + 2) * C + c] + d * d * n;
  }
  mean_out[c] = m;
  invstd[c] = 1.0f / sqrtf(m2 / total + eps);
  if (total_out && c == 0) total_out[0] = total;
  if (running_mean) {
    running_mean[c] = (1.f - momentum) * running_mean[c] + momentum * m;
    running_var[c] = (1.f - momentum) * running_var[c] + momentum * (m2 / (total > 1.f ? total - 1.f : 1.f));
  }
}

inline int bn_cq(int C);
inline int bn_apply_rows(int64_t R, int C);
inline int bn_cq(int C) { const int q = C >> 2; return q >= 64 ? 64 : (q >= 32 ? 32 : (q >= 16 ? 16 : (q >= 8 ? 8 : 4))); }
inline int bn_chunk_rows(int64_t R, int C) {
  const int cq = bn_cq(C), col_blocks = ((C >> 2) + cq - 1) / cq;
  const int64_t target = std::min<int64_t>(1024, std::max<int64_t>(1, 1024 / col_blocks));
  return (int)std::max<int64_t>(128, (R + target - 1) / target);
}
inline int bn_chunks(int64_t R, int C) { const int cr = bn_chunk_rows(R, C); return (int)((R + cr - 1) / cr); }
inline int bn_apply_rows(int64_t R, int C) {
  const int cq = bn_cq(C), col_blocks = ((C >> 2) + cq - 1) / cq, nty = 256 / cq;
  const int64_t rows = (R * col_blocks + 4095) / 4096;
  return (int)std::min<int64_t>(256, std::max<int64_t>(nty, (rows + nty - 1) / nty * nty));
}
inline bool bn_ok(const void* p) { return (reinterpret_cast<uintptr_t>(p) & 15) == 0; }

}
}

using namespace spml;

#define SPML_BN_BY_MASK(KERNEL, MASK, ...)                                        \
  do {                                                                            \
    if ((MASK) == 1) hipLaunchKernelGGL((KERNEL<1>), __VA_ARGS__);                \
    else if ((MASK) == 2) hipLaunchKernelGGL((KERNEL<2>), __VA_ARGS__);           \
    else hipLaunchKernelGGL((KERNEL<0>), __VA_ARGS__);                            \
  } while (0)
#define SPML_BN_PARTIAL1(MASK, ...)                                               \
  do {                                                                            \
    if ((MASK) == 1) hipLaunchKernelGGL((bn_partial<1, 1>), __VA_ARGS__);         \
    else if ((MASK) == 2) hipLaunchKernelGGL((bn_partial<1, 2>), __VA_ARGS__);    \
    else hipLaunchKernelGGL((bn_partial<1, 0>), __VA_ARGS__);                     \
  } while (0)
#define SPML_BN_APPLY(HAS_RES, ...)                                               \
  do {                                                                            \
    if (HAS_RES) hipLaunchKernelGGL((bn_apply<true>), __VA_ARGS__);               \
    else hipLaunchKernelGGL((bn_apply<false>), __VA_ARGS__);                      \
  } while (0)

extern "C" size_t spml_bn_workspace_bytes(int64_t R, int C) {
  if (R <= 0 || C <= 0) return 0;
  return (size_t)4 * bn_chunks(R, C) * C * 4 + 256;
}

extern "C" int spml_bn_stats_f32(const float* x, int64_t R, int C, float* mean, float* m2, void* ws,
                                 size_t ws_bytes, void* stream) {
  if (!x || !mean || !m2 || R <= 0 || C <= 0) return SPML_ERR_INVALID_ARG;
  if ((C & 3) || !bn_ok(x) || !bn_ok(mean) || !bn_ok(m2)) return SPML_ERR_UNSUPPORTED;
  if (!ws || ws_bytes < spml_bn_workspace_bytes(R, C)) return SPML_ERR_WORKSPACE;
  const int chunks = bn_chunks(R, C), cq = bn_cq(C), crows = bn_chunk_rows(R, C);
  float* pa = static_cast<float*>(ws);
  float* pb = pa + (size_t)chunks * C;
  hipStream_t s = (hipStream_t)stream;
  hipLaunchKernelGGL((bn_partial<0, 0>), dim3(((C >> 2) + cq - 1) / cq, chunks), dim3(256), 0, s, x,
                     (const float*)nullptr, (const float*)nullptr, (const float*)nullptr, R, C, cq, crows, pa, pb, (const unsigned char*)nullptr, (float*)nullptr, (float*)nullptr, (float*)nullptr);
  hipLaunchKernelGGL(bn_merge<0>, dim3((C + kMergeCh - 1) / kMergeCh), dim3(kMergeCh * kMergeLanes), 0, s, pa, pb, R, C, chunks, crows,
                     (const float*)nullptr, mean, m2, BnFinal{0, 0.f, 0.f, nullptr, nullptr}, (const float*)nullptr, (const float*)nullptr, (float*)nullptr, (float*)nullptr, BnBound{});
  return launch_status();
}

extern "C" int spml_bn_act_apply_f32(const float* x, const float* residual, int64_t R, int C,
                                     const float* mean, const float* invstd, const float* gamma,
                                     const float* beta, int relu, float* y, void* stream) {
  if (!x || !mean || !invstd || !gamma || !beta || !y || R <= 0 || C <= 0) return SPML_ERR_INVALID_ARG;
  if ((C & 3) || !bn_ok(x) || !bn_ok(y) || (residual && !bn_ok(residual)) || !bn_ok(mean) ||
      !bn_ok(invstd) || !bn_ok(gamma) || !bn_ok(beta))
    return SPML_ERR_UNSUPPORTED;
  const int cq = bn_cq(C), arows = bn_apply_rows(R, C);
  const dim3 grid(((C >> 2) + cq - 1) / cq, (unsigned)((R + arows - 1) / arows));
  SPML_BN_APPLY(residual != nullptr, grid, dim3(256), 0, (hipStream_t)stream, x, residual, R, C, cq, arows, mean, invstd,
                     gamma, beta, relu, y, (uint2*)nullptr, (const float*)nullptr, (unsigned char*)nullptr);
  return launch_status();
}

extern "C" int spml_bn_act_bwd_reduce_f32(const float* dy, const float* y, const float* x, int64_t R,
                                          int C, const float* mean, const float* invstd,
                                          float* sum_dz, float* sum_dz_xhat, void* ws, size_t ws_bytes,
                                          void* stream) {
  if (!dy || !x || !mean || !invstd || !sum_dz || !sum_dz_xhat || R <= 0 || C <= 0)
    return SPML_ERR_INVALID_ARG;
  if ((C & 3) || !bn_ok(dy) || !bn_ok(x) || (y && !bn_ok(y)) || !bn_ok(mean)) return SPML_ERR_UNSUPPORTED;
  if (!ws || ws_bytes < spml_bn_workspace_bytes(R, C)) return SPML_ERR_WORKSPACE;
  const int chunks = bn_chunks(R, C), cq = bn_cq(C), crows = bn_chunk_rows(R, C);
  float* pa = static_cast<float*>(ws);
  float* pb = pa + (size_t)chunks * C;
  hipStream_t s = (hipStream_t)stream;
  SPML_BN_PARTIAL1(y ? 1 : 0, dim3(((C >> 2) + cq - 1) / cq, chunks), dim3(256), 0, s, x, dy, y, mean, R, C, cq, crows,
                   pa, pb, (const unsigned char*)nullptr, (float*)nullptr, (float*)nullptr, (float*)nullptr);
  hipLaunchKernelGGL(bn_merge<1>, dim3((C + kMergeCh - 1) / kMergeCh), dim3(kMergeCh * kMergeLanes), 0, s, pa, pb, R, C, chunks, crows, invstd, sum_dz,
                     sum_dz_xhat, BnFinal{0, 0.f, 0.f, nullptr, nullptr}, (const float*)nullptr, (const float*)nullptr, (float*)nullptr, (float*)nullptr, BnBound{});
  return launch_status();
}

extern "C" int spml_bn_act_bwd_apply_f32(const float* dy, const float* y, const float* x, int64_t R,
                                         int C, const float* mean, const float* invstd,
                                         const float* gamma, const float* sum_dz,
                                         const float* sum_dz_xhat, double count,
                                         const float* count_dev, float* dx,
                                         float* d_residual, void* stream) {
  if (!dy || R <= 0 || C <= 0 || (!dx && !d_residual) || (count <= 0 && !count_dev)) return SPML_ERR_INVALID_ARG;
  if (dx && (!x || !mean || !invstd || !gamma || !sum_dz || !sum_dz_xhat)) return SPML_ERR_INVALID_ARG;
  if ((C & 3) || !bn_ok(dy) || (y && !bn_ok(y)) || (dx && !bn_ok(dx)) || (d_residual && !bn_ok(d_residual)))
    return SPML_ERR_UNSUPPORTED;
  const int cq = bn_cq(C), arows = bn_apply_rows(R, C);
  const dim3 grid(((C >> 2) + cq - 1) / cq, (unsigned)((R + arows - 1) / arows));
  SPML_BN_BY_MASK(bn_bwd_apply, y ? 1 : 0, grid, dim3(256), 0, (hipStream_t)stream, dy, y, x, R, C, cq, arows, mean, invstd,
                     gamma, sum_dz, sum_dz_xhat, count > 0 ? (float)(1.0 / count) : 0.f, count_dev, dx, d_residual,
                     (const unsigned char*)nullptr, (uint2*)nullptr, (const float*)nullptr);
  return launch_status();
}

extern "C" int spml_bn_act_fwd_f32(const float* x, const float* residual, int64_t R, int C,
                                   const float* gamma, const float* beta, float* running_mean,
                                   float* running_var, float momentum, float eps, int relu, float* y,
                                   float* mean, float* invstd, void* ws, size_t ws_bytes,
                                   void* stream) {
  if (!x || !gamma || !beta || !y || !mean || !invstd || R <= 0 || C <= 0) return SPML_ERR_INVALID_ARG;
  if ((C & 3) || !bn_ok(x) || !bn_ok(y) || (residual && !bn_ok(residual)) || !bn_ok(mean) ||
      !bn_ok(invstd) || !bn_ok(gamma) || !bn_ok(beta))
    return SPML_ERR_UNSUPPORTED;
  if (!ws || ws_bytes < spml_bn_workspace_bytes(R, C)) return SPML_ERR_WORKSPACE;
  const int chunks = bn_chunks(R, C), cq = bn_cq(C), crows = bn_chunk_rows(R, C), arows = bn_apply_rows(R, C);
  float* pa = static_cast<float*>(ws);
  float* pb = pa + (size_t)chunks * C;
  hipStream_t s = (hipStream_t)stream;
  hipLaunchKernelGGL((bn_partial<0, 0>), dim3(((C >> 2) + cq - 1) / cq, chunks), dim3(256), 0, s, x,
                     (const float*)nullptr, (const float*)nullptr, (const float*)nullptr, R, C, cq, crows, pa, pb, (const unsigned char*)nullptr, (float*)nullptr, (float*)nullptr, (float*)nullptr);
  hipLaunchKernelGGL(bn_merge<0>, dim3((C + kMergeCh - 1) / kMergeCh), dim3(kMergeCh * kMergeLanes), 0, s, pa, pb, R, C, chunks, crows,
                     (const float*)nullptr, mean, invstd, BnFinal{1, eps, momentum, running_mean, running_var}, (const float*)nullptr, (const float*)nullptr, (float*)nullptr, (float*)nullptr, BnBound{});
  const dim3 grid(((C >> 2) + cq - 1) / cq, (unsigned)((R + arows - 1) / arows));
  SPML_BN_APPLY(residual != nullptr, grid, dim3(256), 0, s, x, residual, R, C, cq, arows, mean, invstd, gamma, beta, relu, y, (uint2*)nullptr, (const float*)nullptr, (unsigned char*)nullptr);
  return launch_status();
}

extern "C" int spml_bn_act_bwd_f32(const float* dy, const float* y, const float* x, int64_t R, int C,
                                   const float* mean, const float* invstd, const float* gamma,
                                   float* d_gamma, float* d_beta, float* dx, float* d_residual,
                                   void* ws, size_t ws_bytes, void* stream) {
  if (!dy || !x || !mean || !invstd || !gamma || !d_gamma || !d_beta || R <= 0 || C <= 0)
    return SPML_ERR_INVALID_ARG;
  int rc = spml_bn_act_bwd_reduce_f32(dy, y, x, R, C, mean, invstd, d_beta, d_gamma, ws, ws_bytes, stream);
  if (rc != SPML_OK) return rc;
  if (!dx && !d_residual) return SPML_OK;
  return spml_bn_act_bwd_apply_f32(dy, y, x, R, C, mean, invstd, gamma, d_beta, d_gamma, (double)R, nullptr, dx,
                                   d_residual, stream);
}

extern "C" int spml_bn_stats_ext_f32(const float* x, int64_t R, int C, float* mean, float* m2, float* cmax,
                                     float* cmin, void* ws, size_t ws_bytes, void* stream) {
  if (!x || !mean || !m2 || !cmax || !cmin || R <= 0 || C <= 0) return SPML_ERR_INVALID_ARG;
  if ((C & 3) || !bn_ok(x) || !bn_ok(mean) || !bn_ok(m2)) return SPML_ERR_UNSUPPORTED;
  if (!ws || ws_bytes < spml_bn_workspace_bytes(R, C)) return SPML_ERR_WORKSPACE;
  const int chunks = bn_chunks(R, C), cq = bn_cq(C), crows = bn_chunk_rows(R, C);
  float* pa = static_cast<float*>(ws);
  float* pb = pa + (size_t)chunks * C;
  float* pc = pb + (size_t)chunks * C;
  float* pd = pc + (size_t)chunks * C;
  hipStream_t s = (hipStream_t)stream;
  hipLaunchKernelGGL((bn_partial<0, 0>), dim3(((C >> 2) + cq - 1) / cq, chunks), dim3(256), 0, s, x,
                     (const float*)nullptr, (const float*)nullptr, (const float*)nullptr, R, C, cq, crows, pa, pb,
                     (const unsigned char*)nullptr, pc, pd, (float*)nullptr);
  hipLaunchKernelGGL(bn_merge<0>, dim3((C + kMergeCh - 1) / kMergeCh), dim3(kMergeCh * kMergeLanes), 0, s, pa, pb, R, C, chunks, crows,
                     (const float*)nullptr, mean, m2, BnFinal{0, 0.f, 0.f, nullptr, nullptr}, (const float*)pc,
                     (const float*)pd, cmax, cmin, BnBound{});
  return launch_status();
}

extern "C" int spml_bn_stats_ext_chunks_f32(const float* chunk_stats, int chunks, int chunk_rows, int64_t R, int C,
                                            float* mean, float* m2, float* cmax, float* cmin, void* stream) {
  if (!chunk_stats || !mean || !m2 || !cmax || !cmin || R <= 0 || C <= 0 || chunks <= 0 || chunk_rows <= 0 ||
      (int64_t)chunks * chunk_rows < R || (int64_t)(chunks - 1) * chunk_rows >= R)
    return SPML_ERR_INVALID_ARG;
  const float* pa = chunk_stats;
  const float* pb = pa + (size_t)chunks * C;
  const float* pc = pb + (size_t)chunks * C;
  const float* pd = pc + (size_t)chunks * C;
  hipLaunchKernelGGL(bn_merge<0>, dim3((C + kMergeCh - 1) / kMergeCh), dim3(kMergeCh * kMergeLanes), 0,
                     (hipStream_t)stream, pa, pb, R, C, chunks, chunk_rows, (const float*)nullptr, mean, m2,
                     BnFinal{0, 0.f, 0.f, nullptr, nullptr}, pc, pd, cmax, cmin, BnBound{});
  return launch_status();
}

extern "C" int spml_bn_finalize_f32(const float* mean, const float* m2, int C, double count, float eps,
                                    float momentum, float* running_mean, float* running_var, float* invstd,
                                    void* stream) {
  if (!mean || !m2 || !invstd || C <= 0 || count <= 0) return SPML_ERR_INVALID_ARG;
  hipLaunchKernelGGL(bn_finalize, dim3((C + 255) / 256), dim3(256), 0, (hipStream_t)stream, C, mean, m2,
                     (float)count, eps, momentum, running_mean, running_var, invstd);
  return launch_status();
}

extern "C" int spml_bn_act_apply_hl8_f32(const float* x, const float* residual, const float* residual_bound,
                                         int64_t R, int C, const float* mean, const float* invstd,
                                         const float* gamma, const float* beta, const float* cmax,
                                         const float* cmin, int relu, float* y, void* y_hl8, float* y_bound,
                                         unsigned char* relu_mask, void* stream) {
  if (!x || !mean || !invstd || !gamma || !beta || (!y && !y_hl8) || R <= 0 || C <= 0) return SPML_ERR_INVALID_ARG;
  if ((y_hl8 || y_bound) && (!cmax || !cmin || !y_bound || (residual && !residual_bound))) return SPML_ERR_INVALID_ARG;
  if ((C & 7) || !bn_ok(x) || (y && !bn_ok(y)) || (y_hl8 && !bn_ok(y_hl8)) || (residual && !bn_ok(residual)) ||
      !bn_ok(mean) || !bn_ok(invstd) || !bn_ok(gamma) || !bn_ok(beta))
    return SPML_ERR_UNSUPPORTED;
  hipStream_t s = (hipStream_t)stream;
  if (y_bound)
    hipLaunchKernelGGL(bn_bound_fwd, dim3(1), dim3(256), 0, s, C, cmax, cmin, mean, invstd, gamma, beta,
                       residual ? residual_bound : (const float*)nullptr, y_bound);
  const int cq = bn_cq(C), arows = bn_apply_rows(R, C);
  const dim3 grid(((C >> 2) + cq - 1) / cq, (unsigned)((R + arows - 1) / arows));
  SPML_BN_APPLY(residual != nullptr, grid, dim3(256), 0, s, x, residual, R, C, cq, arows, mean, invstd, gamma, beta, relu, y,
                static_cast<uint2*>(y_hl8), (const float*)y_bound, relu_mask);
  return launch_status();
}

extern "C" int spml_bn_act_bwd_reduce_ext_f32(const float* dy, const float* y, const unsigned char* relu_mask,
                                              const float* x,
                                              int64_t R, int C, const float* mean, const float* invstd,
                                              float* sum_dz, float* sum_dz_xhat, float* max_dz, void* ws,
                                              size_t ws_bytes, void* stream) {
  if (!dy || !x || !mean || !invstd || !sum_dz || !sum_dz_xhat || !max_dz || R <= 0 || C <= 0)
    return SPML_ERR_INVALID_ARG;
  if ((C & 7) || !bn_ok(dy) || !bn_ok(x) || (y && !bn_ok(y)) || !bn_ok(mean)) return SPML_ERR_UNSUPPORTED;
  if (!ws || ws_bytes < spml_bn_workspace_bytes(R, C)) return SPML_ERR_WORKSPACE;
  const int chunks = bn_chunks(R, C), cq = bn_cq(C), crows = bn_chunk_rows(R, C);
  float* pa = static_cast<float*>(ws);
  float* pb = pa + (size_t)chunks * C;
  float* pc = pb + (size_t)chunks * C;
  hipStream_t s = (hipStream_t)stream;
  SPML_BN_PARTIAL1(y ? 1 : (relu_mask ? 2 : 0), dim3(((C >> 2) + cq - 1) / cq, chunks), dim3(256), 0, s, x, dy, y, mean,
                   R, C, cq, crows, pa, pb, relu_mask, pc, (float*)nullptr, (float*)nullptr);
  hipLaunchKernelGGL(bn_merge<1>, dim3((C + kMergeCh - 1) / kMergeCh), dim3(kMergeCh * kMergeLanes), 0, s, pa, pb, R, C, chunks, crows,
                     invstd, sum_dz, sum_dz_xhat, BnFinal{0, 0.f, 0.f, nullptr, nullptr}, (const float*)pc,
                     (const float*)nullptr, max_dz, (float*)nullptr, BnBound{});
  return launch_status();
}

extern "C" int spml_bn_act_bwd_apply_hl8_f32(const float* dy, const float* y, const unsigned char* relu_mask,
                                             const float* x,
                                             int64_t R, int C, const float* mean, const float* invstd,
                                             const float* gamma, const float* sum_dz, const float* sum_dz_xhat,
                                             const float* max_dz, const float* cmax, const float* cmin,
                                             double count, const float* count_dev, float* dx, void* dx_hl8,
                                             float* dx_bound, float* d_residual, void* stream) {
  if (!dy || R <= 0 || C <= 0 || (!dx && !dx_hl8 && !d_residual) || (count <= 0 && !count_dev))
    return SPML_ERR_INVALID_ARG;
  const float inv_count = count > 0 ? (float)(1.0 / count) : 0.f;
  if ((dx || dx_hl8) && (!x || !mean || !invstd || !gamma || !sum_dz || !sum_dz_xhat)) return SPML_ERR_INVALID_ARG;
  if (dx_hl8 && (!max_dz || !cmax || !cmin || !dx_bound)) return SPML_ERR_INVALID_ARG;
  if ((C & 7) || !bn_ok(dy) || (y && !bn_ok(y)) || (dx && !bn_ok(dx)) ||
      (dx_hl8 && !bn_ok(dx_hl8)) || (d_residual && !bn_ok(d_residual)))
    return SPML_ERR_UNSUPPORTED;
  hipStream_t s = (hipStream_t)stream;
  if (dx_hl8)
    hipLaunchKernelGGL(bn_bound_bwd, dim3(1), dim3(256), 0, s, C, max_dz, cmax, cmin, mean, invstd, gamma, sum_dz,
                       sum_dz_xhat, inv_count, count_dev, dx_bound);
  const int cq = bn_cq(C), arows = bn_apply_rows(R, C);
  const dim3 grid(((C >> 2) + cq - 1) / cq, (unsigned)((R + arows - 1) / arows));
  SPML_BN_BY_MASK(bn_bwd_apply, y ? 1 : (relu_mask ? 2 : 0), grid, dim3(256), 0, s, dy, y, x, R, C, cq, arows, mean, invstd, gamma, sum_dz,
                     sum_dz_xhat, inv_count, count_dev, dx, d_residual, relu_mask,
                  static_cast<uint2*>(dx_hl8), (const float*)dx_bound);
  return launch_status();
}

extern "C" int spml_bn_fwd_hl8_f32(const float* x, const float* residual, const float* residual_bound, int64_t R,
                                   int C, const float* gamma, const float* beta, float* running_mean,
                                   float* running_var, float momentum, float eps, int relu, float* y, void* y_hl8,
                                   float* y_bound, unsigned char* relu_mask, float* mean, float* invstd,
                                   float* cmax, float* cmin, void* ws, size_t ws_bytes, void* stream) {
  if (!x || !gamma || !beta || (!y && !y_hl8) || !y_bound || !mean || !invstd || !cmax || !cmin || R <= 0 || C <= 0 ||
      (residual && !residual_bound))
    return SPML_ERR_INVALID_ARG;
  if ((C & 7) || !bn_ok(x) || (y && !bn_ok(y)) || (y_hl8 && !bn_ok(y_hl8)) || (residual && !bn_ok(residual)) ||
      !bn_ok(mean) || !bn_ok(invstd) || !bn_ok(gamma) || !bn_ok(beta))
    return SPML_ERR_UNSUPPORTED;
  if (!ws || ws_bytes < spml_bn_workspace_bytes(R, C)) return SPML_ERR_WORKSPACE;
  const int chunks = bn_chunks(R, C), cq = bn_cq(C), crows = bn_chunk_rows(R, C), arows = bn_apply_rows(R, C);
  float* pa = static_cast<float*>(ws);
  float* pb = pa + (size_t)chunks * C;
  float* pc = pb + (size_t)chunks * C;
  float* pd = pc + (size_t)chunks * C;
  hipStream_t s = (hipStream_t)stream;
  hipLaunchKernelGGL((bn_partial<0, 0>), dim3(((C >> 2) + cq - 1) / cq, chunks), dim3(256), 0, s, x,
                     (const float*)nullptr, (const float*)nullptr, (const float*)nullptr, R, C, cq, crows, pa, pb,
                     (const unsigned char*)nullptr, pc, pd, y_bound);
  hipLaunchKernelGGL(bn_merge<0>, dim3((C + kMergeCh - 1) / kMergeCh), dim3(kMergeCh * kMergeLanes), 0, s, pa, pb, R,
                     C, chunks, crows, (const float*)nullptr, mean, invstd,
                     BnFinal{1, eps, momentum, running_mean, running_var}, (const float*)pc, (const float*)pd, cmax,
                     cmin, BnBound{y_bound, residual ? residual_bound : nullptr, gamma, beta, nullptr, nullptr, nullptr, 0.f});
  const dim3 grid(((C >> 2) + cq - 1) / cq, (unsigned)((R + arows - 1) / arows));
  SPML_BN_APPLY(residual != nullptr, grid, dim3(256), 0, s, x, residual, R, C, cq, arows, mean, invstd, gamma, beta,
                relu, y, static_cast<uint2*>(y_hl8), (const float*)y_bound, relu_mask);
  return launch_status();
}

extern "C" int spml_bn_fwd_hl8_chunks_f32(const float* x, const float* chunk_stats, int chunks, int chunk_rows,
                                          const float* residual, const float* residual_bound, int64_t R, int C,
                                          const float* gamma, const float* beta, float* running_mean,
                                          float* running_var, float momentum, float eps, int relu, float* y,
                                          void* y_hl8, float* y_bound, unsigned char* relu_mask, float* mean,
                                          float* invstd, float* cmax, float* cmin, void* stream) {
  if (!x || !chunk_stats || !gamma || !beta || (!y && !y_hl8) || !y_bound || !mean || !invstd || !cmax || !cmin ||
      R <= 0 || C <= 0 || chunks <= 0 || chunk_rows <= 0 || (int64_t)chunks * chunk_rows < R ||
      (int64_t)(chunks - 1) * chunk_rows >= R || (residual && !residual_bound))
    return SPML_ERR_INVALID_ARG;
  if ((C & 7) || !bn_ok(x) || (y && !bn_ok(y)) || (y_hl8 && !bn_ok(y_hl8)) || (residual && !bn_ok(residual)) ||
      !bn_ok(mean) || !bn_ok(invstd) || !bn_ok(gamma) || !bn_ok(beta))
    return SPML_ERR_UNSUPPORTED;
  const int cq = bn_cq(C), arows = bn_apply_rows(R, C);
  const float* pa = chunk_stats;
  const float* pb = pa + (size_t)chunks * C;
  const float* pc = pb + (size_t)chunks * C;
  const float* pd = pc + (size_t)chunks * C;
  hipStream_t s = (hipStream_t)stream;
  hipLaunchKernelGGL(bn_merge<0>, dim3((C + kMergeCh - 1) / kMergeCh), dim3(kMergeCh * kMergeLanes), 0, s, pa, pb, R,
                     C, chunks, chunk_rows, (const float*)nullptr, mean, invstd,
                     BnFinal{1, eps, momentum, running_mean, running_var}, pc, pd, cmax, cmin,
                     BnBound{y_bound, residual ? residual_bound : nullptr, gamma, beta, nullptr, nullptr, nullptr, 0.f});
  const dim3 grid(((C >> 2) + cq - 1) / cq, (unsigned)((R + arows - 1) / arows));
  SPML_BN_APPLY(residual != nullptr, grid, dim3(256), 0, s, x, residual, R, C, cq, arows, mean, invstd, gamma, beta,
                relu, y, static_cast<uint2*>(y_hl8), (const float*)y_bound, relu_mask);
  return launch_status();
}

extern "C" int spml_bn_bwd_hl8_f32(const float* dy, const float* y, const unsigned char* relu_mask, const float* x,
                                   int64_t R, int C, const float* mean, const float* invstd, const float* gamma,
                                   const float* cmax, const float* cmin, float* d_gamma, float* d_beta, float* dx,
                                   void* dx_hl8, float* dx_bound, float* d_residual, void* ws, size_t ws_bytes,
                                   void* stream) {
  if (!dy || !x || !mean || !invstd || !gamma || !cmax || !cmin || !d_gamma || !d_beta || R <= 0 || C <= 0 ||
      (dx_hl8 && !dx_bound))
    return SPML_ERR_INVALID_ARG;
  if ((C & 7) || !bn_ok(dy) || !bn_ok(x) || (y && !bn_ok(y)) || (dx && !bn_ok(dx)) || (dx_hl8 && !bn_ok(dx_hl8)) ||
      (d_residual && !bn_ok(d_residual)) || !bn_ok(mean))
    return SPML_ERR_UNSUPPORTED;
  if (!ws || ws_bytes < spml_bn_workspace_bytes(R, C)) return SPML_ERR_WORKSPACE;
  const int chunks = bn_chunks(R, C), cq = bn_cq(C), crows = bn_chunk_rows(R, C), arows = bn_apply_rows(R, C);
  float* pa = static_cast<float*>(ws);
  float* pb = pa + (size_t)chunks * C;
  float* pc = pb + (size_t)chunks * C;
  float* max_dz = pc + (size_t)chunks * C;
  hipStream_t s = (hipStream_t)stream;
  const int mask = y ? 1 : (relu_mask ? 2 : 0);
  SPML_BN_PARTIAL1(mask, dim3(((C >> 2) + cq - 1) / cq, chunks), dim3(256), 0, s, x, dy, y, mean, R, C, cq, crows, pa, pb,
                   relu_mask, pc, (float*)nullptr, dx_hl8 ? dx_bound : (float*)nullptr);
  hipLaunchKernelGGL(bn_merge<1>, dim3((C + kMergeCh - 1) / kMergeCh), dim3(kMergeCh * kMergeLanes), 0, s, pa, pb, R,
                     C, chunks, crows, invstd, d_beta, d_gamma, BnFinal{0, 0.f, 0.f, nullptr, nullptr},
                     (const float*)pc, (const float*)nullptr, max_dz, (float*)nullptr,
                     BnBound{dx_hl8 ? dx_bound : nullptr, nullptr, gamma, nullptr, mean, cmax, cmin, (float)(1.0 / (double)R)});
  if (!dx && !dx_hl8 && !d_residual) return launch_status();
  const dim3 grid(((C >> 2) + cq - 1) / cq, (unsigned)((R + arows - 1) / arows));
  SPML_BN_BY_MASK(bn_bwd_apply, mask, grid, dim3(256), 0, s, dy, y, x, R, C, cq, arows, mean, invstd, gamma,
                  (const float*)d_beta, (const float*)d_gamma, (float)(1.0 / (double)R), (const float*)nullptr, dx,
                  d_residual, relu_mask, static_cast<uint2*>(dx_hl8), (const float*)dx_bound);
  return launch_status();
}

extern "C" int spml_bn_finalize_ranks_f32(const float* stats, int world, int C, float eps, float momentum,
                                          float* running_mean, float* running_var, float* mean, float* invstd,
                                          float* total_count, void* stream) {
  if (!stats || !mean || !invstd || world < 1 || C <= 0) return SPML_ERR_INVALID_ARG;
  hipLaunchKernelGGL(bn_finalize_ranks, dim3((C + 255) / 256), dim3(256), 0, (hipStream_t)stream, C, world, stats, eps,
                     momentum, running_mean, running_var, mean, invstd, total_count);
  return launch_status();
}
```

Measured before the change: 134.9.

## Fuse BN stat merge into partial kernel via last-block ticket and add nontemporal policy

The batch-norm partial-reduction kernel now takes a tail descriptor. The last block to finish in each column group, found with an atomic ticket counter kept in the workspace, performs the cross-chunk merge, writes the bound and updates running stats. This removes the separate bn_merge launch for the hl8 forward and backward paths. The apply kernels also get a policy template that chooses nontemporal loads and stores by tensor size, to reduce cache pollution for streamed data. The cost is release/acquire fences and atomics, serial merge work in one block per column group, and reliance on the ticket words starting at zero (the Python side now zeroes the workspace tail).

Result: no change. 135.9, median of 2 (+0.7%).

```diff
diff --git a/spml_amd/_ffi.py b/spml_amd/_ffi.py
--- a/spml_amd/_ffi.py
+++ b/spml_amd/_ffi.py
@@ -656,6 +656,7 @@
   ws = _bn_ws.get(key)
   if ws is None or ws.numel() < need:
     ws = workspace(need, device)
+    ws[-256:].zero_()
     _bn_ws[key] = ws
   return ws
 
diff --git a/spml_amd/csrc/bn_act.hip b/spml_amd/csrc/bn_act.hip
--- a/spml_amd/csrc/bn_act.hip
+++ b/spml_amd/csrc/bn_act.hip
@@ -3,6 +3,17 @@
 namespace spml {
 namespace {
 
+
+constexpr int kNtLoads = 1, kNtStores = 2;
+template <bool NT>
+__device__ __forceinline__ float4v load_last_use(const float* p) {
+  return NT ? __builtin_nontemporal_load(reinterpret_cast<const float4v*>(p)) : *reinterpret_cast<const float4v*>(p);
+}
+template <bool NT>
+__device__ __forceinline__ void store_far_use(float* p, float4v v) {
+  if (NT) __builtin_nontemporal_store(v, reinterpret_cast<float4v*>(p));
+  else *reinterpret_cast<float4v*>(p) = v;
+}
 
 __device__ __forceinline__ float4v relu_mask_bits(float4v dz, const unsigned char* __restrict__ mask, size_t row,
                                                   int C, int q) {
@@ -42,13 +53,359 @@
   reinterpret_cast<uint4*>(out)[(row * (size_t)(C >> 3) + (q >> 1)) * 2 + (odd ? 1 : 0)] = unit;
 }
 
+struct BnFinal { int fin; float eps, momentum; float* running_mean; float* running_var; };
+struct BnBound {
+  float* bound;
+  const float* res_bound;
+  const float* gamma;
+  const float* beta;
+  const float* mean;
+  const float* cmax;
+  const float* cmin;
+  float inv_count;
+};
+constexpr int kMergeLanes = 64;
+
+__device__ __forceinline__ float chunk_count(int i, int chunk_rows, int64_t R) {
+  return (float)min((int64_t)chunk_rows, R - (int64_t)i * chunk_rows);
+}
+
+struct BnMergeCoef { float gamma, beta, res, rm, rv, is, mu, cmax, cmin; };
+
+template <int MODE>
+__device__ __forceinline__ BnMergeCoef merge_coefficients(int c, const float* __restrict__ invstd, const BnFinal& f,
+                                                          const BnBound& bb) {
+  BnMergeCoef k = {0.f, 0.f, 0.f, 0.f, 0.f, 0.f, 0.f, 0.f, 0.f};
+  if (MODE == 0) {
+    if (f.fin && bb.bound) { k.gamma = bb.gamma[c]; k.beta = bb.beta[c]; k.res = bb.res_bound ? *bb.res_bound : 0.f; }
+    if (f.fin && f.running_mean) { k.rm = f.running_mean[c]; k.rv = f.running_var[c]; }
+  } else {
+    k.is = invstd[c];
+    if (bb.bound) { k.mu = bb.mean[c]; k.cmax = bb.cmax[c]; k.cmin = bb.cmin[c]; k.gamma = bb.gamma[c]; }
+  }
+  return k;
+}
+
+template <int MODE>
+__device__ __forceinline__ unsigned merge_finish(int c, int64_t R, float a, float b, float hi, float lo,
+                                                 const BnMergeCoef& k, float* __restrict__ out_a,
+                                                 float* __restrict__ out_b, const BnFinal& f, const BnBound& bb) {
+  if (MODE == 0) {
+    const float m = a, m2 = b;
+    out_a[c] = m;
+    if (!f.fin) {
+      out_b[c] = m2;
+      return 0u;
+    }
+    const float is = 1.0f / sqrtf(m2 / (float)R + f.eps);
+    out_b[c] = is;
+    if (f.running_mean) {
+      f.running_mean[c] = (1.f - f.momentum) * k.rm + f.momentum * m;
+      f.running_var[c] = (1.f - f.momentum) * k.rv +
+                         f.momentum * (m2 / (float)(R > 1 ? R - 1 : 1));
+    }
+    if (!bb.bound) return 0u;
+    const float sc = k.gamma * is, bt = k.beta;
+    const float v = fmaxf(fabsf((hi - m) * sc + bt), fabsf((lo - m) * sc + bt)) * 1.0001f + k.res;
+    return __float_as_uint(v);
+  } else {
+    const float s0 = a, s1 = b;
+    out_a[c] = s0;
+    out_b[c] = s1 * k.is;
+    if (!bb.bound) return 0u;
+    const float is = k.is, mu = k.mu;
+    const float xh = fmaxf(fabsf(k.cmax - mu), fabsf(k.cmin - mu)) * is;
+    const float v = fabsf(k.gamma * is) *
+                    (hi + fabsf(s0) * bb.inv_count + xh * fabsf(s1 * is) * bb.inv_count) * 1.0001f;
+    return __float_as_uint(v);
+  }
+}
+
+constexpr int kMergeCh = 4;
+
+__device__ inline float merge_lanes(float v, float* sh, int tx, int ty) {
+  __syncthreads();
+  sh[ty * kMergeCh + tx] = v;
+  __syncthreads();
+  float t = 0.f;
+#pragma unroll 16
+  for (int i = 0; i < kMergeLanes; ++i) t += sh[i * kMergeCh + tx];
+  return t;
+}
+
+template <int MODE>
+__global__ __launch_bounds__(kMergeCh * kMergeLanes) void bn_merge(
+    const float* __restrict__ pa, const float* __restrict__ pb, int64_t R, int C, int chunks, int chunk_rows,
+    const float* __restrict__ invstd, float* __restrict__ out_a, float* __restrict__ out_b, BnFinal f,
+    const float* __restrict__ pc, const float* __restrict__ pd, float* __restrict__ out_c,
+    float* __restrict__ out_d, BnBound bb) {
+  __shared__ float sh[kMergeCh * kMergeLanes];
+  __shared__ float sh_bound[kMergeCh];
+  const int tx = threadIdx.x % kMergeCh, ty = threadIdx.x / kMergeCh;
+  const int n_live = min(kMergeCh, C - (int)blockIdx.x * kMergeCh);
+  auto publish_bound = [&](float v) {
+    sh_bound[tx] = v;
+    __builtin_amdgcn_wave_barrier();
+    if (tx == 0) {
+      unsigned m = __float_as_uint(v);
+      for (int i = 1; i < n_live; ++i) m = max(m, __float_as_uint(sh_bound[i]));
+      atomicMax(reinterpret_cast<unsigned*>(bb.bound), m);
+    }
+  };
+  const int c = min(blockIdx.x * kMergeCh + tx, C - 1);
+  const bool live = blockIdx.x * kMergeCh + tx < C && ty == 0;
+  float hi = -3.4e38f, lo = 3.4e38f;
+  constexpr int kMergeRegs = 16;
+  const bool in_regs = chunks <= kMergeRegs * kMergeLanes;
+  const bool ext = pc && out_c;
+  float ra[kMergeRegs], rb[kMergeRegs], rc[kMergeRegs], rd[kMergeRegs];
+  if (in_regs) {
+#pragma unroll
+    for (int j = 0; j < kMergeRegs; ++j) {
+      const int i = ty + j * kMergeLanes;
+      const bool ok = i < chunks;
+      const size_t o = (size_t)(ok ? i : 0) * C + c;
+      ra[j] = ok ? pa[o] : 0.f;
+      rb[j] = ok ? pb[o] : 0.f;
+      rc[j] = (ok && ext) ? pc[o] : -3.4e38f;
+      rd[j] = (ok && ext && MODE == 0) ? pd[o] : 3.4e38f;
+    }
+  }
+  float p_gamma = 0.f, p_beta = 0.f, p_res = 0.f, p_rm = 0.f, p_rv = 0.f, p_is = 0.f, p_mu = 0.f, p_cmax = 0.f, p_cmin = 0.f;
+  if (live) {
+    if (MODE == 0) {
+      if (f.fin && bb.bound) { p_gamma = bb.gamma[c]; p_beta = bb.beta[c]; p_res = bb.res_bound ? *bb.res_bound : 0.f; }
+      if (f.fin && f.running_mean) { p_rm = f.running_mean[c]; p_rv = f.running_var[c]; }
+    } else {
+      p_is = invstd[c];
+      if (bb.bound) { p_mu = bb.mean[c]; p_cmax = bb.cmax[c]; p_cmin = bb.cmin[c]; p_gamma = bb.gamma[c]; }
+    }
+  }
+  if (ext) {
+    if (in_regs) {
+#pragma unroll
+      for (int j = 0; j < kMergeRegs; ++j) {
+        hi = fmaxf(hi, rc[j]);
+        if (MODE == 0) lo = fminf(lo, rd[j]);
+      }
+    } else {
+#pragma unroll 4
+      for (int i = ty; i < chunks; i += kMergeLanes) {
+        hi = fmaxf(hi, pc[(size_t)i * C + c]);
+        if (MODE == 0) lo = fminf(lo, pd[(size_t)i * C + c]);
+      }
+    }
+    __syncthreads();
+    sh[ty * kMergeCh + tx] = hi;
+    __syncthreads();
+    for (int i = 0; i < kMergeLanes; ++i) hi = fmaxf(hi, sh[i * kMergeCh + tx]);
+    if (MODE == 0) {
+      __syncthreads();
+      sh[ty * kMergeCh + tx] = lo;
+      __syncthreads();
+      for (int i = 0; i < kMergeLanes; ++i) lo = fminf(lo, sh[i * kMergeCh + tx]);
+    }
+    if (live) {
+      out_c[c] = hi;
+      if (MODE == 0) out_d[c] = lo;
+    }
+  }
+  if (MODE == 0) {
+    float sm = 0.f;
+    if (in_regs) {
+#pragma unroll
+      for (int j = 0; j < kMergeRegs; ++j) {
+        const int i = ty + j * kMergeLanes;
+        if (i < chunks) {
+          const float nb = (float)min((int64_t)chunk_rows, R - (int64_t)i * chunk_rows);
+          sm += ra[j] * nb;
+        }
+      }
+    } else {
+#pragma unroll 4
+      for (int i = ty; i < chunks; i += kMergeLanes) {
+        const float nb = (float)min((int64_t)chunk_rows, R - (int64_t)i * chunk_rows);
+        sm += pa[(size_t)i * C + c] * nb;
+      }
+    }
+    const float m = merge_lanes(sm, sh, tx, ty) / (float)R;
+    float m2 = 0.f;
+    if (in_regs) {
+#pragma unroll
+      for (int j = 0; j < kMergeRegs; ++j) {
+        const int i = ty + j * kMergeLanes;
+        if (i < chunks) {
+          const float nb = (float)min((int64_t)chunk_rows, R - (int64_t)i * chunk_rows);
+          const float d = ra[j] - m;
+          m2 += rb[j] + d * d * nb;
+        }
+      }
+    } else {
+#pragma unroll 4
+      for (int i = ty; i < chunks; i += kMergeLanes) {
+        const float nb = (float)min((int64_t)chunk_rows, R - (int64_t)i * chunk_rows);
+        const float d = pa[(size_t)i * C + c] - m;
+        m2 += pb[(size_t)i * C + c] + d * d * nb;
+      }
+    }
+    m2 = merge_lanes(m2, sh, tx, ty);
+    if (!live) return;
+    out_a[c] = m;
+    if (f.fin) {
+      const float is = 1.0f / sqrtf(m2 / (float)R + f.eps);
+      out_b[c] = is;
+      if (bb.bound) {
+        const float sc = p_gamma * is, b = p_beta;
+        const float v = fmaxf(fabsf((hi - m) * sc + b), fabsf((lo - m) * sc + b)) * 1.0001f + p_res;
+        publish_bound(v);
+      }
+      if (f.running_mean) {
+        f.running_mean[c] = (1.f - f.momentum) * p_rm + f.momentum * m;
+        f.running_var[c] = (1.f - f.momentum) * p_rv +
+                           f.momentum * (m2 / (float)(R > 1 ? R - 1 : 1));
+      }
+    } else {
+      out_b[c] = m2;
+    }
+  } else {
+    float s0 = 0.f, s1 = 0.f;
+    if (in_regs) {
+#pragma unroll
+      for (int j = 0; j < kMergeRegs; ++j)
+        if (ty + j * kMergeLanes < chunks) { s0 += ra[j]; s1 += rb[j]; }
+    } else {
+      for (int i = ty; i < chunks; i += kMergeLanes) { s0 += pa[(size_t)i * C + c]; s1 += pb[(size_t)i * C + c]; }
+    }
+    s0 = merge_lanes(s0, sh, tx, ty);
+    s1 = merge_lanes(s1, sh, tx, ty);
+    if (!live) return;
+    out_a[c] = s0;
+    out_b[c] = s1 * p_is;
+    if (bb.bound) {
+      const float is = p_is, mu = p_mu;
+      const float xh = fmaxf(fabsf(p_cmax - mu), fabsf(p_cmin - mu)) * is;
+      const float v = fabsf(p_gamma * is) *
+                      (hi + fabsf(s0) * bb.inv_count + xh * fabsf(s1 * is) * bb.inv_count) * 1.0001f;
+      publish_bound(v);
+    }
+  }
+}
+
+struct BnTail {
+  unsigned* tickets;
+  const float* invstd;
+  float* out_a;
+  float* out_b;
+  float* out_c;
+  float* out_d;
+  BnFinal f;
+  BnBound bb;
+};
+constexpr int kTailWords = 64, kTailFinal = 62, kTailBound = 63, kTailMaxColBlocks = 62;
+
+template <int MODE>
+__device__ __forceinline__ float tail_fold(float v, float* sh, int W, int G, int cx, int g, float t) {
+  __syncthreads();
+  sh[g * W + cx] = v;
+  __syncthreads();
+  if (g == 0)
+    for (int i = 0; i < G; ++i) t += sh[i * W + cx];
+  return t;
+}
+
+template <int MODE>
+__device__ void bn_tail_merge(float* sh, const float* pa, const float* pb, const float* pc, const float* pd, int64_t R,
+                              int C, int chunks, int chunk_rows, int c0, int W, const BnTail& tl) {
+  const int G = 256 / W, cx = threadIdx.x % W, g = threadIdx.x / W;
+  const int c = min(c0 + cx, C - 1);
+  const bool live = g == 0 && c0 + cx < C;
+  const bool ext = pc && tl.out_c;
+  BnMergeCoef coef = {0.f, 0.f, 0.f, 0.f, 0.f, 0.f, 0.f, 0.f, 0.f};
+  if (live) coef = merge_coefficients<MODE>(c, tl.invstd, tl.f, tl.bb);
+  float hi = -3.4e38f, lo = 3.4e38f, a = 0.f, b = 0.f;
+  for (int l = g; l < kMergeLanes; l += G) {
+    float s0 = 0.f, s1 = 0.f;
+#pragma unroll 4
+    for (int i = l; i < chunks; i += kMergeLanes) {
+      const size_t o = (size_t)i * C + c;
+      if (MODE == 0) {
+        const float nb = chunk_count(i, chunk_rows, R);
+        s0 += pa[o] * nb;
+      } else {
+        s0 += pa[o];
+        s1 += pb[o];
+      }
+      if (ext) {
+        hi = fmaxf(hi, pc[o]);
+        if (MODE == 0) lo = fminf(lo, pd[o]);
+      }
+    }
+    a = tail_fold<MODE>(s0, sh, W, G, cx, g, a);
+    if (MODE == 1) b = tail_fold<MODE>(s1, sh, W, G, cx, g, b);
+  }
+  if (MODE == 0) {
+    __syncthreads();
+    if (g == 0) sh[512 + cx] = a / (float)R;
+    __syncthreads();
+    const float m = sh[512 + cx];
+    for (int l = g; l < kMergeLanes; l += G) {
+      float m2 = 0.f;
+#pragma unroll 4
+      for (int i = l; i < chunks; i += kMergeLanes) {
+        const size_t o = (size_t)i * C + c;
+        const float nb = chunk_count(i, chunk_rows, R);
+        const float d = pa[o] - m;
+        m2 += pb[o] + d * d * nb;
+      }
+      b = tail_fold<MODE>(m2, sh, W, G, cx, g, b);
+    }
+    a = m;
+  }
+  if (ext) {
+    __syncthreads();
+    sh[g * W + cx] = hi;
+    sh[256 + g * W + cx] = lo;
+    __syncthreads();
+    for (int i = 0; i < G; ++i) {
+      hi = fmaxf(hi, sh[i * W + cx]);
+      lo = fminf(lo, sh[256 + i * W + cx]);
+    }
+    if (live) {
+      tl.out_c[c] = hi;
+      if (MODE == 0) tl.out_d[c] = lo;
+    }
+  }
+  unsigned v = live ? merge_finish<MODE>(c, R, a, b, hi, lo, coef, tl.out_a, tl.out_b, tl.f, tl.bb) : 0u;
+  if (!tl.bb.bound) return;
+#pragma unroll
+  for (int o = 32; o > 0; o >>= 1) v = max(v, (unsigned)__shfl_xor((int)v, o, kWave));
+  unsigned* shu = reinterpret_cast<unsigned*>(sh);
+  __syncthreads();
+  if ((threadIdx.x & 63) == 0) shu[threadIdx.x >> 6] = v;
+  __syncthreads();
+  if (threadIdx.x != 0) return;
+  v = max(max(shu[0], shu[1]), max(shu[2], shu[3]));
+  if (gridDim.x > 1) {
+    __hip_atomic_fetch_max(tl.tickets + kTailBound, v, __ATOMIC_RELAXED, __HIP_MEMORY_SCOPE_AGENT);
+    __builtin_amdgcn_fence(__ATOMIC_RELEASE, "agent");
+    asm volatile("s_waitcnt vmcnt(0)" ::: "memory");
+    const unsigned t = __hip_atomic_fetch_add(tl.tickets + kTailFinal, 1u, __ATOMIC_RELAXED, __HIP_MEMORY_SCOPE_AGENT);
+    if (t + 1 != gridDim.x) return;
+    __builtin_amdgcn_fence(__ATOMIC_ACQUIRE, "agent");
+    asm volatile("s_waitcnt vmcnt(0)" ::: "memory");
+    v = __hip_atomic_exchange(tl.tickets + kTailBound, 0u, __ATOMIC_RELAXED, __HIP_MEMORY_SCOPE_AGENT);
+    __hip_atomic_store(tl.tickets + kTailFinal, 0u, __ATOMIC_RELAXED, __HIP_MEMORY_SCOPE_AGENT);
+  }
+  *reinterpret_cast<unsigned*>(tl.bb.bound) = v;
+}
+
 template <int MODE, int MASK>
 __global__ __launch_bounds__(256) void bn_partial(const float* __restrict__ x, const float* __restrict__ dy,
                                                   const float* __restrict__ y, const float* __restrict__ mean,
                                                   int64_t R, int C, int cq, int chunk_rows,
                                                   float* __restrict__ pa, float* __restrict__ pb,
                                                   const unsigned char* __restrict__ yh, float* __restrict__ pc,
-                                                  float* __restrict__ pd, float* __restrict__ zero_me) {
+                                                  float* __restrict__ pd, float* __restrict__ zero_me, BnTail tl) {
   if (zero_me && blockIdx.x == 0 && blockIdx.y == 0 && threadIdx.x == 0) *zero_me = 0.f;
   __shared__ float4v sa[256], sb[256];
   const int tx = threadIdx.x % cq, ty = threadIdx.x / cq, nty = 256 / cq;
@@ -122,191 +479,31 @@
       if (MODE == 0) *reinterpret_cast<float4v*>(pd + (size_t)blockIdx.y * C + 4 * q) = lo;
     }
   }
-}
-
-struct BnFinal { int fin; float eps, momentum; float* running_mean; float* running_var; };
-struct BnBound {
-  float* bound;
-  const float* res_bound;
-  const float* gamma;
-  const float* beta;
-  const float* mean;
-  const float* cmax;
-  const float* cmin;
-  float inv_count;
-};
-constexpr int kMergeLanes = 64, kMergeCh = 4;
-
-__device__ inline float merge_lanes(float v, float* sh, int tx, int ty) {
+  if (!tl.tickets) return;
+  asm volatile("s_waitcnt vmcnt(0)" ::: "memory");
   __syncthreads();
-  sh[ty * kMergeCh + tx] = v;
+  unsigned* last_flag = reinterpret_cast<unsigned*>(sa);
+  if (threadIdx.x == 0) {
+    __builtin_amdgcn_fence(__ATOMIC_RELEASE, "agent");
+    asm volatile("s_waitcnt vmcnt(0)" ::: "memory");
+    const unsigned t = __hip_atomic_fetch_add(tl.tickets + blockIdx.x, 1u, __ATOMIC_RELAXED, __HIP_MEMORY_SCOPE_AGENT);
+    const bool last = t + 1 == gridDim.y;
+    if (last) {
+      __hip_atomic_store(tl.tickets + blockIdx.x, 0u, __ATOMIC_RELAXED, __HIP_MEMORY_SCOPE_AGENT);
+      __builtin_amdgcn_fence(__ATOMIC_ACQUIRE, "agent");
+      asm volatile("s_waitcnt vmcnt(0)" ::: "memory");
+    }
+    last_flag[0] = last ? 1u : 0u;
+  }
   __syncthreads();
-  float t = 0.f;
-#pragma unroll 16
-  for (int i = 0; i < kMergeLanes; ++i) t += sh[i * kMergeCh + tx];
-  return t;
-}
-
-template <int MODE>
-__global__ __launch_bounds__(kMergeCh * kMergeLanes) void bn_merge(
-    const float* __restrict__ pa, const float* __restrict__ pb, int64_t R, int C, int chunks, int chunk_rows,
-    const float* __restrict__ invstd, float* __restrict__ out_a, float* __restrict__ out_b, BnFinal f,
-    const float* __restrict__ pc, const float* __restrict__ pd, float* __restrict__ out_c,
-    float* __restrict__ out_d, BnBound bb) {
-  __shared__ float sh[kMergeCh * kMergeLanes];
-  __shared__ float sh_bound[kMergeCh];
-  const int tx = threadIdx.x % kMergeCh, ty = threadIdx.x / kMergeCh;
-  const int n_live = min(kMergeCh, C - (int)blockIdx.x * kMergeCh);
-  auto publish_bound = [&](float v) {
-    sh_bound[tx] = v;
-    __builtin_amdgcn_wave_barrier();
-    if (tx == 0) {
-      unsigned m = __float_as_uint(v);
-      for (int i = 1; i < n_live; ++i) m = max(m, __float_as_uint(sh_bound[i]));
-      atomicMax(reinterpret_cast<unsigned*>(bb.bound), m);
-    }
-  };
-  const int c = min(blockIdx.x * kMergeCh + tx, C - 1);
-  const bool live = blockIdx.x * kMergeCh + tx < C && ty == 0;
-  float hi = -3.4e38f, lo = 3.4e38f;
-  constexpr int kMergeRegs = 16;
-  const bool in_regs = chunks <= kMergeRegs * kMergeLanes;
-  const bool ext = pc && out_c;
-  float ra[kMergeRegs], rb[kMergeRegs], rc[kMergeRegs], rd[kMergeRegs];
-  if (in_regs) {
-#pragma unroll
-    for (int j = 0; j < kMergeRegs; ++j) {
-      const int i = ty + j * kMergeLanes;
-      const bool ok = i < chunks;
-      const size_t o = (size_t)(ok ? i : 0) * C + c;
-      ra[j] = ok ? pa[o] : 0.f;
-      rb[j] = ok ? pb[o] : 0.f;
-      rc[j] = (ok && ext) ? pc[o] : -3.4e38f;
-      rd[j] = (ok && ext && MODE == 0) ? pd[o] : 3.4e38f;
-    }
-  }
-  float p_gamma = 0.f, p_beta = 0.f, p_res = 0.f, p_rm = 0.f, p_rv = 0.f, p_is = 0.f, p_mu = 0.f, p_cmax = 0.f, p_cmin = 0.f;
-  if (live) {
-    if (MODE == 0) {
-      if (f.fin && bb.bound) { p_gamma = bb.gamma[c]; p_beta = bb.beta[c]; p_res = bb.res_bound ? *bb.res_bound : 0.f; }
-      if (f.fin && f.running_mean) { p_rm = f.running_mean[c]; p_rv = f.running_var[c]; }
-    } else {
-      p_is = invstd[c];
-      if (bb.bound) { p_mu = bb.mean[c]; p_cmax = bb.cmax[c]; p_cmin = bb.cmin[c]; p_gamma = bb.gamma[c]; }
-    }
-  }
-  if (ext) {
-    if (in_regs) {
-#pragma unroll
-      for (int j = 0; j < kMergeRegs; ++j) {
-        hi = fmaxf(hi, rc[j]);
-        if (MODE == 0) lo = fminf(lo, rd[j]);
-      }
-    } else {
-#pragma unroll 4
-      for (int i = ty; i < chunks; i += kMergeLanes) {
-        hi = fmaxf(hi, pc[(size_t)i * C + c]);
-        if (MODE == 0) lo = fminf(lo, pd[(size_t)i * C + c]);
-      }
-    }
-    __syncthreads();
-    sh[ty * kMergeCh + tx] = hi;
-    __syncthreads();
-    for (int i = 0; i < kMergeLanes; ++i) hi = fmaxf(hi, sh[i * kMergeCh + tx]);
-    if (MODE == 0) {
-      __syncthreads();
-      sh[ty * kMergeCh + tx] = lo;
-      __syncthreads();
-      for (int i = 0; i < kMergeLanes; ++i) lo = fminf(lo, sh[i * kMergeCh + tx]);
-    }
-    if (live) {
-      out_c[c] = hi;
-      if (MODE == 0) out_d[c] = lo;
-    }
-  }
-  if (MODE == 0) {
-    float sm = 0.f;
-    if (in_regs) {
-#pragma unroll
-      for (int j = 0; j < kMergeRegs; ++j) {
-        const int i = ty + j * kMergeLanes;
-        if (i < chunks) {
-          const float nb = (float)min((int64_t)chunk_rows, R - (int64_t)i * chunk_rows);
-          sm += ra[j] * nb;
-        }
-      }
-    } else {
-#pragma unroll 4
-      for (int i = ty; i < chunks; i += kMergeLanes) {
-        const float nb = (float)min((int64_t)chunk_rows, R - (int64_t)i * chunk_rows);
-        sm += pa[(size_t)i * C + c] * nb;
-      }
-    }
-    const float m = merge_lanes(sm, sh, tx, ty) / (float)R;
-    float m2 = 0.f;
-    if (in_regs) {
-#pragma unroll
-      for (int j = 0; j < kMergeRegs; ++j) {
-        const int i = ty + j * kMergeLanes;
-        if (i < chunks) {
-          const float nb = (float)min((int64_t)chunk_rows, R - (int64_t)i * chunk_rows);
-          const float d = ra[j] - m;
-          m2 += rb[j] + d * d * nb;
-        }
-      }
-    } else {
-#pragma unroll 4
-      for (int i = ty; i < chunks; i += kMergeLanes) {
-        const float nb = (float)min((int64_t)chunk_rows, R - (int64_t)i * chunk_rows);
-        const float d = pa[(size_t)i * C + c] - m;
-        m2 += pb[(size_t)i * C + c] + d * d * nb;
-      }
-    }
-    m2 = merge_lanes(m2, sh, tx, ty);
-    if (!live) return;
-    out_a[c] = m;
-    if (f.fin) {
-      const float is = 1.0f / sqrtf(m2 / (float)R + f.eps);
-      out_b[c] = is;
-      if (bb.bound) {
-        const float sc = p_gamma * is, b = p_beta;
-        const float v = fmaxf(fabsf((hi - m) * sc + b), fabsf((lo - m) * sc + b)) * 1.0001f + p_res;
-        publish_bound(v);
-      }
-      if (f.running_mean) {
-        f.running_mean[c] = (1.f - f.momentum) * p_rm + f.momentum * m;
-        f.running_var[c] = (1.f - f.momentum) * p_rv +
-                           f.momentum * (m2 / (float)(R > 1 ? R - 1 : 1));
-      }
-    } else {
-      out_b[c] = m2;
-    }
-  } else {
-    float s0 = 0.f, s1 = 0.f;
-    if (in_regs) {
-#pragma unroll
-      for (int j = 0; j < kMergeRegs; ++j)
-        if (ty + j * kMergeLanes < chunks) { s0 += ra[j]; s1 += rb[j]; }
-    } else {
-      for (int i = ty; i < chunks; i += kMergeLanes) { s0 += pa[(size_t)i * C + c]; s1 += pb[(size_t)i * C + c]; }
-    }
-    s0 = merge_lanes(s0, sh, tx, ty);
-    s1 = merge_lanes(s1, sh, tx, ty);
-    if (!live) return;
-    out_a[c] = s0;
-    out_b[c] = s1 * p_is;
-    if (bb.bound) {
-      const float is = p_is, mu = p_mu;
-      const float xh = fmaxf(fabsf(p_cmax - mu), fabsf(p_cmin - mu)) * is;
-      const float v = fabsf(p_gamma * is) *
-                      (hi + fabsf(s0) * bb.inv_count + xh * fabsf(s1 * is) * bb.inv_count) * 1.0001f;
-      publish_bound(v);
-    }
-  }
-}
-
-
-template <bool HAS_RES>
+  const bool last = last_flag[0] != 0u;
+  if (!last) return;
+  bn_tail_merge<MODE>(reinterpret_cast<float*>(sa), pa, pb, pc, pd, R, C, (int)gridDim.y, chunk_rows,
+                      (int)blockIdx.x * cq * 4, cq * 4, tl);
+}
+
+
+template <bool HAS_RES, int POLICY>
 __global__ __launch_bounds__(256) void bn_apply(const float* __restrict__ x, const float* __restrict__ res,
                                                 int64_t R, int C, int cq, int apply_rows,
                                                 const float* __restrict__ mean,
@@ -324,18 +521,18 @@
   const float4v sc = *reinterpret_cast<const float4v*>(invstd + 4 * q) *
                      *reinterpret_cast<const float4v*>(gamma + 4 * q);
   const float4v sh = *reinterpret_cast<const float4v*>(beta + 4 * q);
-  const int64_t r0 = (int64_t)blockIdx.y * apply_rows;
+  const int64_t r0 = (int64_t)(gridDim.y - 1 - blockIdx.y) * apply_rows;
   const int64_t r1 = min(R, r0 + apply_rows);
 #pragma unroll 4
   for (int64_t r = r0 + ty; r < r1; r += nty) {
     const size_t o = (size_t)r * C + 4 * q;
-    float4v v = (*reinterpret_cast<const float4v*>(x + o) - mu) * sc + sh;
-    if (HAS_RES) v += *reinterpret_cast<const float4v*>(res + o);
+    float4v v = (load_last_use<(POLICY & kNtLoads) != 0>(x + o) - mu) * sc + sh;
+    if (HAS_RES) v += load_last_use<(POLICY & kNtLoads) != 0>(res + o);
     if (relu) {
 #pragma unroll
       for (int e = 0; e < 4; ++e) v[e] = fmaxf(v[e], 0.f);
     }
-    if (y) *reinterpret_cast<float4v*>(y + o) = v;
+    if (y) store_far_use<(POLICY & kNtStores) != 0>(y + o, v);
     if (yh) store_hl8_quad(yh, (size_t)r, C, q, v, ys);
     if (mask)
       mask[(size_t)r * (C >> 2) + q] = (unsigned char)((v[0] > 0.f) | ((v[1] > 0.f) << 1) | ((v[2] > 0.f) << 2) |
@@ -343,7 +540,7 @@
   }
 }
 
-template <int MASK>
+template <int MASK, int POLICY>
 __global__ __launch_bounds__(256) void bn_bwd_apply(const float* __restrict__ dy, const float* __restrict__ y,
                                                     const float* __restrict__ x, int64_t R, int C, int cq,
                                                     int apply_rows, const float* __restrict__ mean,
@@ -368,12 +565,12 @@
     c0 = *reinterpret_cast<const float4v*>(sum_dz + 4 * q) * inv_count;
     c1 = *reinterpret_cast<const float4v*>(sum_dz_xhat + 4 * q) * inv_count;
   }
-  const int64_t r0 = (int64_t)blockIdx.y * apply_rows;
+  const int64_t r0 = (int64_t)(gridDim.y - 1 - blockIdx.y) * apply_rows;
   const int64_t r1 = min(R, r0 + apply_rows);
 #pragma unroll 4
   for (int64_t r = r0 + ty; r < r1; r += nty) {
     const size_t o = (size_t)r * C + 4 * q;
-    float4v dz = *reinterpret_cast<const float4v*>(dy + o);
+    float4v dz = load_last_use<(POLICY & kNtLoads) != 0>(dy + o);
     if (MASK == 1) {
       const float4v yv = *reinterpret_cast<const float4v*>(y + o);
 #pragma unroll
@@ -381,9 +578,9 @@
     } else if (MASK == 2) {
       dz = relu_mask_bits(dz, yh, (size_t)r, C, q);
     }
-    if (dres) *reinterpret_cast<float4v*>(dres + o) = dz;
+    if (dres) store_far_use<(POLICY & kNtStores) != 0>(dres + o, dz);
     if (dx || dxh) {
-      const float4v xh = (*reinterpret_cast<const float4v*>(x + o) - mu) * is;
+      const float4v xh = (load_last_use<(POLICY & kNtLoads) != 0>(x + o) - mu) * is;
       const float4v g = gi * (dz - c0 - xh * c1);
       if (dx) *reinterpret_cast<float4v*>(dx + o) = g;
       if (dxh) store_hl8_quad(dxh, (size_t)r, C, q, g, ds);
@@ -491,23 +688,45 @@
   return (int)std::max<int64_t>(128, (R + target - 1) / target);
 }
 inline int bn_chunks(int64_t R, int C) { const int cr = bn_chunk_rows(R, C); return (int)((R + cr - 1) / cr); }
+constexpr int kApplyBlocks = 8192;
 inline int bn_apply_rows(int64_t R, int C) {
   const int cq = bn_cq(C), col_blocks = ((C >> 2) + cq - 1) / cq, nty = 256 / cq;
-  const int64_t rows = (R * col_blocks + 4095) / 4096;
+  const int64_t rows = (R * col_blocks + kApplyBlocks - 1) / kApplyBlocks;
   return (int)std::min<int64_t>(256, std::max<int64_t>(nty, (rows + nty - 1) / nty * nty));
 }
 inline bool bn_ok(const void* p) { return (reinterpret_cast<uintptr_t>(p) & 15) == 0; }
+inline int bn_policy(int64_t R, int C, bool far_stores) {
+  return ((size_t)R * C * 4 >= ((size_t)128 << 20) ? kNtLoads : 0) | (far_stores ? kNtStores : 0);
+}
+constexpr size_t kTailMaxBytes = 64 << 10;
+inline bool bn_tail_ok(int C, int chunks) {
+  const int cq = bn_cq(C), col_blocks = ((C >> 2) + cq - 1) / cq;
+  const size_t bytes = (size_t)chunks * std::min(4 * cq, C) * 16;
+  return col_blocks <= kTailMaxColBlocks && bytes <= kTailMaxBytes;
+}
+inline unsigned* bn_tickets(void* ws, size_t ws_bytes) {
+  return reinterpret_cast<unsigned*>(static_cast<char*>(ws) + ((ws_bytes - 4 * kTailWords) & ~(size_t)3));
+}
 
 }
 }
 
 using namespace spml;
 
-#define SPML_BN_BY_MASK(KERNEL, MASK, ...)                                        \
-  do {                                                                            \
-    if ((MASK) == 1) hipLaunchKernelGGL((KERNEL<1>), __VA_ARGS__);                \
-    else if ((MASK) == 2) hipLaunchKernelGGL((KERNEL<2>), __VA_ARGS__);           \
-    else hipLaunchKernelGGL((KERNEL<0>), __VA_ARGS__);                            \
+#define SPML_BN_BY_POLICY(POLICY, KERNEL, FIRST, ...)                                            \
+  do {                                                                                           \
+    switch (POLICY) {                                                                            \
+      case 1: hipLaunchKernelGGL((KERNEL<FIRST, 1>), __VA_ARGS__); break;                        \
+      case 2: hipLaunchKernelGGL((KERNEL<FIRST, 2>), __VA_ARGS__); break;                        \
+      case 3: hipLaunchKernelGGL((KERNEL<FIRST, 3>), __VA_ARGS__); break;                        \
+      default: hipLaunchKernelGGL((KERNEL<FIRST, 0>), __VA_ARGS__);                              \
+    }                                                                                            \
+  } while (0)
+#define SPML_BN_BWD_APPLY(MASK, POLICY, ...)                                                     \
+  do {                                                                                           \
+    if ((MASK) == 1) SPML_BN_BY_POLICY(POLICY, bn_bwd_apply, 1, __VA_ARGS__);                    \
+    else if ((MASK) == 2) SPML_BN_BY_POLICY(POLICY, bn_bwd_apply, 2, __VA_ARGS__);               \
+    else SPML_BN_BY_POLICY(POLICY, bn_bwd_apply, 0, __VA_ARGS__);                                \
   } while (0)
 #define SPML_BN_PARTIAL1(MASK, ...)                                               \
   do {                                                                            \
@@ -515,10 +734,10 @@
     else if ((MASK) == 2) hipLaunchKernelGGL((bn_partial<1, 2>), __VA_ARGS__);    \
     else hipLaunchKernelGGL((bn_partial<1, 0>), __VA_ARGS__);                     \
   } while (0)
-#define SPML_BN_APPLY(HAS_RES, ...)                                               \
-  do {                                                                            \
-    if (HAS_RES) hipLaunchKernelGGL((bn_apply<true>), __VA_ARGS__);               \
-    else hipLaunchKernelGGL((bn_apply<false>), __VA_ARGS__);                      \
+#define SPML_BN_APPLY(HAS_RES, POLICY, ...)                                                      \
+  do {                                                                                           \
+    if (HAS_RES) SPML_BN_BY_POLICY(POLICY, bn_apply, true, __VA_ARGS__);                         \
+    else SPML_BN_BY_POLICY(POLICY, bn_apply, false, __VA_ARGS__);                                \
   } while (0)
 
 extern "C" size_t spml_bn_workspace_bytes(int64_t R, int C) {
@@ -536,7 +755,7 @@
   float* pb = pa + (size_t)chunks * C;
   hipStream_t s = (hipStream_t)stream;
   hipLaunchKernelGGL((bn_partial<0, 0>), dim3(((C >> 2) + cq - 1) / cq, chunks), dim3(256), 0, s, x,
-                     (const float*)nullptr, (const float*)nullptr, (const float*)nullptr, R, C, cq, crows, pa, pb, (const unsigned char*)nullptr, (float*)nullptr, (float*)nullptr, (float*)nullptr);
+                     (const float*)nullptr, (const float*)nullptr, (const float*)nullptr, R, C, cq, crows, pa, pb, (const unsigned char*)nullptr, (float*)nullptr, (float*)nullptr, (float*)nullptr, BnTail{});
   hipLaunchKernelGGL(bn_merge<0>, dim3((C + kMergeCh - 1) / kMergeCh), dim3(kMergeCh * kMergeLanes), 0, s, pa, pb, R, C, chunks, crows,
                      (const float*)nullptr, mean, m2, BnFinal{0, 0.f, 0.f, nullptr, nullptr}, (const float*)nullptr, (const float*)nullptr, (float*)nullptr, (float*)nullptr, BnBound{});
   return launch_status();
@@ -551,7 +770,7 @@
     return SPML_ERR_UNSUPPORTED;
   const int cq = bn_cq(C), arows = bn_apply_rows(R, C);
   const dim3 grid(((C >> 2) + cq - 1) / cq, (unsigned)((R + arows - 1) / arows));
-  SPML_BN_APPLY(residual != nullptr, grid, dim3(256), 0, (hipStream_t)stream, x, residual, R, C, cq, arows, mean, invstd,
+  SPML_BN_APPLY(residual != nullptr, bn_policy(R, C, false), grid, dim3(256), 0, (hipStream_t)stream, x, residual, R, C, cq, arows, mean, invstd,
                      gamma, beta, relu, y, (uint2*)nullptr, (const float*)nullptr, (unsigned char*)nullptr);
   return launch_status();
 }
@@ -569,7 +788,7 @@
   float* pb = pa + (size_t)chunks * C;
   hipStream_t s = (hipStream_t)stream;
   SPML_BN_PARTIAL1(y ? 1 : 0, dim3(((C >> 2) + cq - 1) / cq, chunks), dim3(256), 0, s, x, dy, y, mean, R, C, cq, crows,
-                   pa, pb, (const unsigned char*)nullptr, (float*)nullptr, (float*)nullptr, (float*)nullptr);
+                   pa, pb, (const unsigned char*)nullptr, (float*)nullptr, (float*)nullptr, (float*)nullptr, BnTail{});
   hipLaunchKernelGGL(bn_merge<1>, dim3((C + kMergeCh - 1) / kMergeCh), dim3(kMergeCh * kMergeLanes), 0, s, pa, pb, R, C, chunks, crows, invstd, sum_dz,
                      sum_dz_xhat, BnFinal{0, 0.f, 0.f, nullptr, nullptr}, (const float*)nullptr, (const float*)nullptr, (float*)nullptr, (float*)nullptr, BnBound{});
   return launch_status();
@@ -587,7 +806,7 @@
     return SPML_ERR_UNSUPPORTED;
   const int cq = bn_cq(C), arows = bn_apply_rows(R, C);
   const dim3 grid(((C >> 2) + cq - 1) / cq, (unsigned)((R + arows - 1) / arows));
-  SPML_BN_BY_MASK(bn_bwd_apply, y ? 1 : 0, grid, dim3(256), 0, (hipStream_t)stream, dy, y, x, R, C, cq, arows, mean, invstd,
+  SPML_BN_BWD_APPLY(y ? 1 : 0, bn_policy(R, C, false), grid, dim3(256), 0, (hipStream_t)stream, dy, y, x, R, C, cq, arows, mean, invstd,
                      gamma, sum_dz, sum_dz_xhat, count > 0 ? (float)(1.0 / count) : 0.f, count_dev, dx, d_residual,
                      (const unsigned char*)nullptr, (uint2*)nullptr, (const float*)nullptr);
   return launch_status();
@@ -608,11 +827,11 @@
   float* pb = pa + (size_t)chunks * C;
   hipStream_t s = (hipStream_t)stream;
   hipLaunchKernelGGL((bn_partial<0, 0>), dim3(((C >> 2) + cq - 1) / cq, chunks), dim3(256), 0, s, x,
-                     (const float*)nullptr, (const float*)nullptr, (const float*)nullptr, R, C, cq, crows, pa, pb, (const unsigned char*)nullptr, (float*)nullptr, (float*)nullptr, (float*)nullptr);
+                     (const float*)nullptr, (const float*)nullptr, (const float*)nullptr, R, C, cq, crows, pa, pb, (const unsigned char*)nullptr, (float*)nullptr, (float*)nullptr, (float*)nullptr, BnTail{});
   hipLaunchKernelGGL(bn_merge<0>, dim3((C + kMergeCh - 1) / kMergeCh), dim3(kMergeCh * kMergeLanes), 0, s, pa, pb, R, C, chunks, crows,
                      (const float*)nullptr, mean, invstd, BnFinal{1, eps, momentum, running_mean, running_var}, (const float*)nullptr, (const float*)nullptr, (float*)nullptr, (float*)nullptr, BnBound{});
   const dim3 grid(((C >> 2) + cq - 1) / cq, (unsigned)((R + arows - 1) / arows));
-  SPML_BN_APPLY(residual != nullptr, grid, dim3(256), 0, s, x, residual, R, C, cq, arows, mean, invstd, gamma, beta, relu, y, (uint2*)nullptr, (const float*)nullptr, (unsigned char*)nullptr);
+  SPML_BN_APPLY(residual != nullptr, bn_policy(R, C, false), grid, dim3(256), 0, s, x, residual, R, C, cq, arows, mean, invstd, gamma, beta, relu, y, (uint2*)nullptr, (const float*)nullptr, (unsigned char*)nullptr);
   return launch_status();
 }
 
@@ -642,7 +861,7 @@
   hipStream_t s = (hipStream_t)stream;
   hipLaunchKernelGGL((bn_partial<0, 0>), dim3(((C >> 2) + cq - 1) / cq, chunks), dim3(256), 0, s, x,
                      (const float*)nullptr, (const float*)nullptr, (const float*)nullptr, R, C, cq, crows, pa, pb,
-                     (const unsigned char*)nullptr, pc, pd, (float*)nullptr);
+                     (const unsigned char*)nullptr, pc, pd, (float*)nullptr, BnTail{});
   hipLaunchKernelGGL(bn_merge<0>, dim3((C + kMergeCh - 1) / kMergeCh), dim3(kMergeCh * kMergeLanes), 0, s, pa, pb, R, C, chunks, crows,
                      (const float*)nullptr, mean, m2, BnFinal{0, 0.f, 0.f, nullptr, nullptr}, (const float*)pc,
                      (const float*)pd, cmax, cmin, BnBound{});
@@ -689,7 +908,7 @@
                        residual ? residual_bound : (const float*)nullptr, y_bound);
   const int cq = bn_cq(C), arows = bn_apply_rows(R, C);
   const dim3 grid(((C >> 2) + cq - 1) / cq, (unsigned)((R + arows - 1) / arows));
-  SPML_BN_APPLY(residual != nullptr, grid, dim3(256), 0, s, x, residual, R, C, cq, arows, mean, invstd, gamma, beta, relu, y,
+  SPML_BN_APPLY(residual != nullptr, bn_policy(R, C, y && y_hl8), grid, dim3(256), 0, s, x, residual, R, C, cq, arows, mean, invstd, gamma, beta, relu, y,
                 static_cast<uint2*>(y_hl8), (const float*)y_bound, relu_mask);
   return launch_status();
 }
@@ -709,7 +928,7 @@
   float* pc = pb + (size_t)chunks * C;
   hipStream_t s = (hipStream_t)stream;
   SPML_BN_PARTIAL1(y ? 1 : (relu_mask ? 2 : 0), dim3(((C >> 2) + cq - 1) / cq, chunks), dim3(256), 0, s, x, dy, y, mean,
-                   R, C, cq, crows, pa, pb, relu_mask, pc, (float*)nullptr, (float*)nullptr);
+                   R, C, cq, crows, pa, pb, relu_mask, pc, (float*)nullptr, (float*)nullptr, BnTail{});
   hipLaunchKernelGGL(bn_merge<1>, dim3((C + kMergeCh - 1) / kMergeCh), dim3(kMergeCh * kMergeLanes), 0, s, pa, pb, R, C, chunks, crows,
                      invstd, sum_dz, sum_dz_xhat, BnFinal{0, 0.f, 0.f, nullptr, nullptr}, (const float*)pc,
                      (const float*)nullptr, max_dz, (float*)nullptr, BnBound{});
@@ -737,7 +956,7 @@
                        sum_dz_xhat, inv_count, count_dev, dx_bound);
   const int cq = bn_cq(C), arows = bn_apply_rows(R, C);
   const dim3 grid(((C >> 2) + cq - 1) / cq, (unsigned)((R + arows - 1) / arows));
-  SPML_BN_BY_MASK(bn_bwd_apply, y ? 1 : (relu_mask ? 2 : 0), grid, dim3(256), 0, s, dy, y, x, R, C, cq, arows, mean, invstd, gamma, sum_dz,
+  SPML_BN_BWD_APPLY(y ? 1 : (relu_mask ? 2 : 0), bn_policy(R, C, true), grid, dim3(256), 0, s, dy, y, x, R, C, cq, arows, mean, invstd, gamma, sum_dz,
                      sum_dz_xhat, inv_count, count_dev, dx, d_residual, relu_mask,
                   static_cast<uint2*>(dx_hl8), (const float*)dx_bound);
   return launch_status();
@@ -761,15 +980,18 @@
   float* pc = pb + (size_t)chunks * C;
   float* pd = pc + (size_t)chunks * C;
   hipStream_t s = (hipStream_t)stream;
+  const bool tail = bn_tail_ok(C, chunks);
+  const BnFinal fin{1, eps, momentum, running_mean, running_var};
+  const BnBound bb{y_bound, residual ? residual_bound : nullptr, gamma, beta, nullptr, nullptr, nullptr, 0.f};
   hipLaunchKernelGGL((bn_partial<0, 0>), dim3(((C >> 2) + cq - 1) / cq, chunks), dim3(256), 0, s, x,
                      (const float*)nullptr, (const float*)nullptr, (const float*)nullptr, R, C, cq, crows, pa, pb,
-                     (const unsigned char*)nullptr, pc, pd, y_bound);
-  hipLaunchKernelGGL(bn_merge<0>, dim3((C + kMergeCh - 1) / kMergeCh), dim3(kMergeCh * kMergeLanes), 0, s, pa, pb, R,
-                     C, chunks, crows, (const float*)nullptr, mean, invstd,
-                     BnFinal{1, eps, momentum, running_mean, running_var}, (const float*)pc, (const float*)pd, cmax,
-                     cmin, BnBound{y_bound, residual ? residual_bound : nullptr, gamma, beta, nullptr, nullptr, nullptr, 0.f});
+                     (const unsigned char*)nullptr, pc, pd, tail ? (float*)nullptr : y_bound,
+                     tail ? BnTail{bn_tickets(ws, ws_bytes), nullptr, mean, invstd, cmax, cmin, fin, bb} : BnTail{});
+  if (!tail)
+    hipLaunchKernelGGL(bn_merge<0>, dim3((C + kMergeCh - 1) / kMergeCh), dim3(kMergeCh * kMergeLanes), 0, s, pa, pb, R, C, chunks, crows,
+                       (const float*)nullptr, mean, invstd, fin, (const float*)pc, (const float*)pd, cmax, cmin, bb);
   const dim3 grid(((C >> 2) + cq - 1) / cq, (unsigned)((R + arows - 1) / arows));
-  SPML_BN_APPLY(residual != nullptr, grid, dim3(256), 0, s, x, residual, R, C, cq, arows, mean, invstd, gamma, beta,
+  SPML_BN_APPLY(residual != nullptr, bn_policy(R, C, y && y_hl8), grid, dim3(256), 0, s, x, residual, R, C, cq, arows, mean, invstd, gamma, beta,
                 relu, y, static_cast<uint2*>(y_hl8), (const float*)y_bound, relu_mask);
   return launch_status();
 }
@@ -798,7 +1020,7 @@
                      BnFinal{1, eps, momentum, running_mean, running_var}, pc, pd, cmax, cmin,
                      BnBound{y_bound, residual ? residual_bound : nullptr, gamma, beta, nullptr, nullptr, nullptr, 0.f});
   const dim3 grid(((C >> 2) + cq - 1) / cq, (unsigned)((R + arows - 1) / arows));
-  SPML_BN_APPLY(residual != nullptr, grid, dim3(256), 0, s, x, residual, R, C, cq, arows, mean, invstd, gamma, beta,
+  SPML_BN_APPLY(residual != nullptr, bn_policy(R, C, y && y_hl8), grid, dim3(256), 0, s, x, residual, R, C, cq, arows, mean, invstd, gamma, beta,
                 relu, y, static_cast<uint2*>(y_hl8), (const float*)y_bound, relu_mask);
   return launch_status();
 }
@@ -822,15 +1044,18 @@
   float* max_dz = pc + (size_t)chunks * C;
   hipStream_t s = (hipStream_t)stream;
   const int mask = y ? 1 : (relu_mask ? 2 : 0);
+  const bool tail = bn_tail_ok(C, chunks);
+  const BnFinal fin{0, 0.f, 0.f, nullptr, nullptr};
+  const BnBound bb{dx_hl8 ? dx_bound : nullptr, nullptr, gamma, nullptr, mean, cmax, cmin, (float)(1.0 / (double)R)};
   SPML_BN_PARTIAL1(mask, dim3(((C >> 2) + cq - 1) / cq, chunks), dim3(256), 0, s, x, dy, y, mean, R, C, cq, crows, pa, pb,
-                   relu_mask, pc, (float*)nullptr, dx_hl8 ? dx_bound : (float*)nullptr);
-  hipLaunchKernelGGL(bn_merge<1>, dim3((C + kMergeCh - 1) / kMergeCh), dim3(kMergeCh * kMergeLanes), 0, s, pa, pb, R,
-                     C, chunks, crows, invstd, d_beta, d_gamma, BnFinal{0, 0.f, 0.f, nullptr, nullptr},
-                     (const float*)pc, (const float*)nullptr, max_dz, (float*)nullptr,
-                     BnBound{dx_hl8 ? dx_bound : nullptr, nullptr, gamma, nullptr, mean, cmax, cmin, (float)(1.0 / (double)R)});
+                   relu_mask, pc, (float*)nullptr, (dx_hl8 && !tail) ? dx_bound : (float*)nullptr,
+                   tail ? BnTail{bn_tickets(ws, ws_bytes), invstd, d_beta, d_gamma, max_dz, nullptr, fin, bb} : BnTail{});
+  if (!tail)
+    hipLaunchKernelGGL(bn_merge<1>, dim3((C + kMergeCh - 1) / kMergeCh), dim3(kMergeCh * kMergeLanes), 0, s, pa, pb, R, C, chunks, crows,
+                       invstd, d_beta, d_gamma, fin, (const float*)pc, (const float*)nullptr, max_dz, (float*)nullptr, bb);
   if (!dx && !dx_hl8 && !d_residual) return launch_status();
   const dim3 grid(((C >> 2) + cq - 1) / cq, (unsigned)((R + arows - 1) / arows));
-  SPML_BN_BY_MASK(bn_bwd_apply, mask, grid, dim3(256), 0, s, dy, y, x, R, C, cq, arows, mean, invstd, gamma,
+  SPML_BN_BWD_APPLY(mask, bn_policy(R, C, true), grid, dim3(256), 0, s, dy, y, x, R, C, cq, arows, mean, invstd, gamma,
                   (const float*)d_beta, (const float*)d_gamma, (float)(1.0 / (double)R), (const float*)nullptr, dx,
                   d_residual, relu_mask, static_cast<uint2*>(dx_hl8), (const float*)dx_bound);
   return launch_status();
```
